# TIXhjq/ML_Function

Hardware: AMD Instinct MI355X
Metric: samples/sec fwd+bwd xDeepFM-CIN B=4096,F=39,K=16 (higher is better)
Workload: dtype f32

## Files before the change

ml_function_amd/csrc/cin.hip:

```cpp
#include "cin_layout.h"

namespace fil {

static const char* kFwdNames[kCinMaxL] = {"cin_fwd_l1", "cin_fwd_l2", "cin_fwd_l3", "cin_fwd_l4", "cin_fwd_l5", "cin_fwd_l6", "cin_fwd_l7", "cin_fwd_l8"};
static const char* kDwNames[kCinMaxL] = {"cin_bwd_dw_l1", "cin_bwd_dw_l2", "cin_bwd_dw_l3", "cin_bwd_dw_l4", "cin_bwd_dw_l5", "cin_bwd_dw_l6", "cin_bwd_dw_l7", "cin_bwd_dw_l8"};
static const char* kDzNames[kCinMaxL] = {"cin_bwd_dz_l1", "cin_bwd_dz_l2", "cin_bwd_dz_l3", "cin_bwd_dz_l4", "cin_bwd_dz_l5", "cin_bwd_dz_l6", "cin_bwd_dz_l7", "cin_bwd_dz_l8"};
static double gemm_flops(long M, int Hp, int F, int H) { return 2.0 * (double)M * Hp * F * H; }

static int launch_dw3(hipStream_t st, const DwPlan& p, const float* gT, int HS, const float* xT, const float* xpT, int xps, float* part,
                      long M, int F, int Hp, int H, int symD = 0, int xtra = 0) {
  const int items = p.blocks_x * p.splits * p.chunks;
  const dim3 grid((items + 7) / 8 * 8);
#define FIL_DW3(MBV, ONES) \
  hipLaunchKernelGGL((cin_dw3_kernel<MBV, ONES>), grid, dim3(kCinThreads), 0, st, gT, HS, xT, xpT, xps, part, (int)M, F, Hp, H, p.rows_per_split, \
                     p.blocks_x, p.chunks, items, symD, xtra)
  if (xT == nullptr) {
    if (p.MB == 2) FIL_DW3(2, true); else FIL_DW3(1, true);
  } else {
    if (p.MB == 2) FIL_DW3(2, false); else FIL_DW3(1, false);
  }
#undef FIL_DW3
  return p.splits;
}

constexpr int kCinRetiredBits = 0;
static bool tail_used(const CinShape& s, int mode) {
  if ((mode & (FIL_CIN_GENERAL | FIL_CIN_NOTAIL)) != 0) return false;
  const TailGeom g = tail_geom(s);
  if (!g.on) return false;
  return (mode & FIL_CIN_TAIL_ALWAYS) != 0 || 4 * g.JP <= 3 * g.Hq;
}
static bool qtail_used(const CinShape& s, int mode, const CinTune& tune) {
  if (s.M() <= 16384 && (mode & FIL_CIN_TAIL_ALWAYS) == 0) return false;
  return tail_used(s, mode) && s.L == 3 && tune.sym && s.F >= 2 && s.F + 2 <= kQtConst && s.H[0] <= 128 && 3 * s.F + 1 <= s.HSmax() && (mode & FIL_CIN_NOQTAIL) == 0 &&
         knobs().qtail != 0;
}
static bool qmerge_used(const CinShape& s, int mode, const CinTune& tune) {
  return qtail_used(s, mode, tune) && 3 * s.F + 3 <= s.HSmax() && (mode & FIL_CIN_NOQMERGE) == 0 && knobs().qmerge != 0;
}
constexpr int kCinPrecBf16 = 1 << 20;
static bool qsplit_fwd_menu(int JT) { return JT >= 2 && JT <= 12 && JT % 2 == 0; }
static bool qsplit_used(const CinShape& s, int mode, const CinTune& tune) {
  return (mode & (FIL_CIN_BF16X3 | kCinPrecBf16)) != 0 && qmerge_used(s, mode, tune) && knobs().fwdq != 0 && knobs().dz2 != 0 && s.HS(0) == 128 &&
         qsplit_fwd_menu(cin_jt_sym(s.F));
}

struct CinPath {
  bool xt_in;
  bool general;
  bool tail;
  bool qtail;
  bool qmerge;
  bool qsplit;
  int qnp;
  CinTune tune;
  TailGeom tg;
  bool fwdq(const CinShape& s) const { return qmerge && knobs().fwdq != 0 && s.HS(0) == 128; }
};
static CinPath cin_path_of(const CinShape& s, int mode) {
  const CinTune tune(mode);
  return CinPath{(mode & FIL_CIN_X_TRANSPOSED) != 0, (mode & FIL_CIN_GENERAL) != 0, tail_used(s, mode), qtail_used(s, mode, tune), qmerge_used(s, mode, tune),
                 qsplit_used(s, mode, tune), (mode & kCinPrecBf16) != 0 ? 1 : 3, tune, tail_geom(s)};
}
static int cin_precision_bits(const char* who, int mode, int precision, int* bits) {
  if (precision != FIL_CIN_PREC_DEFAULT && precision != FIL_CIN_PREC_BF16)
    return fail(FIL_ERR_ARG, "%s: precision %d (0 DEFAULT, 1 BF16)", who, precision);
  if (precision == FIL_CIN_PREC_BF16 && (mode & FIL_CIN_BF16X3) != 0)
    return fail(FIL_ERR_ARG, "%s: precision BF16 with mode bit BF16X3 (mode %d): two operand precisions", who, mode);
  *bits = precision == FIL_CIN_PREC_BF16 ? kCinPrecBf16 : 0;
  return FIL_OK;
}
static int cin_path(const char* who, const CinShape& s, int mode, int precision, CinPath* path) {
  if (mode < 0 || mode > 1023 || (mode & kCinRetiredBits) != 0)
    return fail(FIL_ERR_UNSUPPORTED, "%s: mode %d (bits: 1 general kernels, 2 BF16X3, 4 MB2, 8 NOSYM, 16 X_TRANSPOSED, 32 NOTAIL, 64 TAIL_ALWAYS, 128 NOKSPLIT, 256 NOQTAIL, 512 NOQMERGE)", who, mode);
  int bits = 0;
  if (int rc = cin_precision_bits(who, mode, precision, &bits)) return rc;
  *path = cin_path_of(s, mode | bits);
  return FIL_OK;
}
static int cin_ready_order(int L, const CinPath& p, int* slot, int* point) {
  int n = 0, pt = 0;
  slot[n] = L, point[n++] = pt;
  if (p.qmerge) slot[n] = 0, point[n++] = pt;
  ++pt;
  int l = L - 1;
  if (p.tail) {
    slot[n] = L - 1, point[n++] = pt;
    slot[n] = L - 2, point[n++] = pt++;
    l = L - 3;
  }
  for (; l >= (p.qmerge ? 1 : 0); --l) slot[n] = l, point[n++] = pt++;
  return pt;
}
static SavedForm saved_form(const CinPath& p) { return p.qtail ? SavedForm::qtail : (p.tail ? SavedForm::tail : SavedForm::plain); }

template <typename KernelT>
static void allow_lds(KernelT kernel, size_t sh) {
  if (sh > 48 * 1024) (void)hipFuncSetAttribute(reinterpret_cast<const void*>(kernel), hipFuncAttributeMaxDynamicSharedMemorySize, (int)sh);
}

struct DzsShape {
  int MBs, ks;
  dim3 grid;
};
static DzsShape dzs_launch_shape(const CinTune& tune, long M, int JTs, int NHMAX) {
  const bool two_waves = NHMAX == 64 && cin_dzs_two_waves(JTs) && tune.mb_forced != 2 && knobs().dzs_mb != 2;
  const int MBs = (two_waves || NHMAX == 128) ? 1 : tune.mb_rows(M);
  const int ks = (NHMAX != 64 || MBs != 1) ? 1 : tune.ksplit(M);
  return DzsShape{MBs, ks, dim3(ks == 4 ? cdiv((int)M, 32) : cdiv((int)M, 128 * MBs))};
}

}

using namespace fil;

extern "C" size_t fil_cin_saved_bytes(int B, int F, int K, int L, const int* H) {
  CinShape s;
  if (check_shape("fil_cin_saved_bytes", B, F, K, L, H, s) != FIL_OK || B == 0) return 0;
  return saved_bytes(s);
}

extern "C" size_t fil_cin_fwd_workspace_bytes(int B, int F, int K, int L, const int* H) {
  CinShape s;
  if (check_shape("fil_cin_fwd_workspace_bytes", B, F, K, L, H, s) != FIL_OK || B == 0) return 0;
  return fwd_ws_bytes(s);
}

extern "C" size_t fil_cin_bwd_workspace_bytes(int B, int F, int K, int L, const int* H) {
  CinShape s;
  if (check_shape("fil_cin_bwd_workspace_bytes", B, F, K, L, H, s) != FIL_OK || B == 0) return 0;
  return bwd_ws_bytes(s);
}

extern "C" int fil_cin_grad_ready_points(int B, int F, int K, int L, const int* H, int mode, int* point) {
  CinShape s;
  if (int rc = check_shape("fil_cin_grad_ready_points", B, F, K, L, H, s)) return rc;
  if (point == nullptr || mode < 0 || mode > 1023) return fail(FIL_ERR_ARG, "fil_cin_grad_ready_points: point == NULL or mode %d out of range", mode);
  if ((mode & kCinRetiredBits) != 0) return fail(FIL_ERR_UNSUPPORTED, "fil_cin_grad_ready_points: mode %d holds a retired bit (2: the split-bf16 experiment)", mode);
  if (B == 0) {
    for (int i = 0; i <= L; ++i) point[i] = 0;
    return 1;
  }
  int slot[kCinMaxL + 1], pt[kCinMaxL + 1];
  const int n = cin_ready_order(L, cin_path_of(s, mode), slot, pt);
  for (int i = 0; i <= L; ++i) point[slot[i]] = pt[i];
  return n;
}

extern "C" int fil_cin_precision_used(int B, int F, int K, int L, const int* H, int mode, int precision) {
  CinShape s;
  if (int rc = check_shape("fil_cin_precision_used", B, F, K, L, H, s)) return rc;
  if (mode < 0 || mode > 1023 || (mode & kCinRetiredBits) != 0) return fail(FIL_ERR_UNSUPPORTED, "fil_cin_precision_used: mode %d", mode);
  int bits = 0;
  if (int rc = cin_precision_bits("fil_cin_precision_used", mode, precision, &bits)) return rc;
  if (bits == 0 || B == 0) return FIL_CIN_PREC_DEFAULT;
  return cin_path_of(s, mode | bits).qsplit ? FIL_CIN_PREC_BF16 : FIL_CIN_PREC_DEFAULT;
}

#define FIL_CIN_CHECK_ARG(cond)                                                          \
  do {                                                                                   \
    if (!(cond)) return ::fil::fail(FIL_ERR_ARG, "%s: bad argument: %s", c.who, #cond); \
  } while (0)
#define FIL_CIN_FWD_LAUNCHED() FIL_CHECK_LAUNCH_W("cin_fwd_impl")
#define FIL_CIN_BWD_LAUNCHED() FIL_CHECK_LAUNCH_W("cin_bwd_impl")

struct CinCall {
  const char* who;
  CinShape s;
  CinPath p;
  hipStream_t st;
  const float* x;
  const float* xT;
  const float* const* W;
  const float* const* bias;
  const float* dense_w;
  int output_dim;
  CinSaved sv;
};
struct CinFwd : CinCall {
  const float* dense_b;
  float *out, *pooled;
  CinFwdWs ws;
  PoolArgs pa;
  const float* xpT;
  bool fused_last = false;
  bool head_done = false;
};

static int cin_fwd_prepare(CinFwd& c) {
  const CinShape& s = c.s;
  const TailGeom& tg = c.p.tg;
  const int B = s.B, F = s.F, K = s.K, L = s.L, JT = s.JT(), XL = cin_x2_len(F);
  const long M = s.M();
  const bool xt_in = c.p.xt_in, need_x2 = c.p.tune.sym;
  hipStream_t st = c.st;
  if (c.p.qtail) {
    FIL_CIN_CHECK_ARG(c.W[0] && c.W[L - 1] && c.W[L - 2]);
    ProfScope ps("cin_fwd_prep", st, 2.0 * M * F * sizeof(float));
    const int JTs = cin_jt_sym(F), chunks0 = chunks_of(s.H[0]);
    const long npack = (long)chunks0 * F * 2 * JTs * 128;
    const bool fq = c.p.fwdq(s);
    const int nt = fq ? 0 : B, npk = (int)std::min<long>((npack + 255) / 256, 1024), nwl = cdiv(tg.Hq * F, 8), nwp = cdiv(tg.Hpp * F, 8);
    const size_t sh = (xt_in || fq) ? 0 : (size_t)F * (K + 1) * sizeof(float);
    allow_lds(cin_qtail_prep_kernel, sh);
    hipLaunchKernelGGL(cin_qtail_prep_kernel, dim3(nt + npk + nwl + nwp), dim3(256), sh, st, c.x, c.sv.xT, F, K, nt, c.W[0], c.ws.Wf, s.H[0], 2 * JTs, chunks0, npk,
                       c.W[L - 1], c.sv.wsumL, tg.Hq, tg.HL, nwl, c.W[L - 2], c.sv.wsumP, c.sv.wsnP, tg.Hpp, 2 * JT, chunks_of(tg.Hpp), c.ws.x2T, XL, xt_in ? 1 : 0);
  } else if (c.p.tail && c.p.tune.sym) {
    FIL_CIN_CHECK_ARG(c.W[0] && c.W[L - 1]);
    ProfScope ps("cin_fwd_prep", st, 2.0 * M * F * sizeof(float));
    const int JTs = cin_jt_sym(F), chunks0 = chunks_of(s.H[0]);
    const long npack = (long)chunks0 * F * 2 * JTs * 128;
    const int nt = B, npk = (int)std::min<long>((npack + 255) / 256, 1024), nws = cdiv(tg.Hq * F, 8), nz = 64;
    const size_t sh = xt_in ? 0 : (size_t)F * (K + 1) * sizeof(float);
    allow_lds(cin_fwd_prep_kernel, sh);
    hipLaunchKernelGGL(cin_fwd_prep_kernel, dim3(nt + npk + nws + nz), dim3(256), sh, st, c.x, c.sv.xT, F, K, nt, c.W[0], c.ws.Wf, s.H[0], 2 * JTs, chunks0,
                       npk, c.W[L - 1], c.sv.bmT, tg.Hq, tg.HL, nws, reinterpret_cast<float4*>(c.sv.Uz), (long)((tg.uz_floats + tg.uf_floats) / 4), c.ws.x2T, XL,
                       xt_in ? 1 : 0);
  } else if (!xt_in || need_x2) {
    ProfScope ps("cin_transpose_in", st, 2.0 * M * F * sizeof(float));
    hipLaunchKernelGGL(cin_transpose_in_kernel, dim3(B), dim3(256), xt_in ? 0 : (size_t)F * (K + 1) * sizeof(float), st, c.x, c.sv.xT, F, K,
                       need_x2 ? c.ws.x2T : nullptr, XL, xt_in ? 1 : 0);
  }
  FIL_CIN_FWD_LAUNCHED();
  return FIL_OK;
}

static int cin_fwd_merged_q(CinFwd& c) {
  const CinShape& s = c.s;
  const TailGeom& tg = c.p.tg;
  const CinSaved& sv = c.sv;
  const CinFwdWs& ws = c.ws;
  const int B = s.B, F = s.F, K = s.K, L = s.L, JT = s.JT(), XL = cin_x2_len(F), *H = s.H;
  const long M = s.M();
  const bool xt_in = c.p.xt_in, qsplit = c.p.qsplit;
  const float* x = c.x;
  hipStream_t st = c.st;
  const int p = tg.p, lL = L - 1, Hpp = tg.Hpp, Hq = tg.Hq, HS0 = s.HS(0);
  FIL_CIN_CHECK_ARG(c.W[p] && c.W[lL] && c.bias[p] && c.bias[lL]);
  const int JTs = cin_jt_sym(F), chunks = chunks_of(Hpp);
  float* x1T = sv.maps[0];
  {
    ProfScope ps("cin_tail_prep", st);
    int ks = -1;
    if (!xt_in && K <= 64 && (K & (K - 1)) == 0 && (reinterpret_cast<uintptr_t>(x) & 15) == 0)
      for (ks = 0; (1 << ks) < K;) ++ks;
    const size_t sh_x = ks >= 0 ? (size_t)(64 >> ks) * F * (K + 1) : (xt_in ? (size_t)64 * (F | 1) : (size_t)F * (K + 1));
    const int tiles = cin_slot_tiles(F, JTs);
    const bool fold = !qsplit && knobs().packfold != 0;
    const QtPackFold pf = fold ? QtPackFold{ws.WfT, sv.WzT, JTs, chunks, HS0, tiles} : QtPackFold{nullptr, nullptr, 0, 0, 0, 0};
    const size_t sh = std::max(cin_qtail_t_lds_floats(F, Hq, fold), sh_x) * sizeof(float);
    allow_lds(cin_qtail_t_x_kernel, sh);
    const int nx = (ks >= 0 || xt_in) ? (int)((M + 63) / 64) : B, nT = cin_qtail_t_wgs(Hpp);
    hipLaunchKernelGGL(cin_qtail_t_x_kernel, dim3(nT + nx), dim3(256), sh, st, c.W[p], sv.wsumL, c.bias[p], c.bias[lL], tg.HL, sv.T, sv.cvec, ws.zbias, Hpp, F, Hq,
                       nT, x, sv.xT, K, ws.x2T, XL, xt_in ? 1 : 0, ks, (ks >= 0 || xt_in) ? (long)M : 0L, pf);
    if (!fold) {
      const long npack = (long)chunks * F * 2 * JTs * 128;
      const int nbf = (int)std::min<long>((npack + 255) / 256, 1024), nbz = (int)std::min<long>(((long)tiles * 32 * HS0 + 255) / 256, 1024);
      const int NTq = qsplit ? cin_qs_steps(F, JTs) : 0, nbq = qsplit ? std::min(cdiv(NTq * 512, 256), 512) : 0;
      if (c.p.qnp == 1)
        hipLaunchKernelGGL(cin_qtail_pack_kernel<1>, dim3(nbf + nbz + nbq), dim3(256), 0, st, sv.T, ws.WfT, sv.WzT, F, Hpp, JTs, chunks, nbf, HS0, tiles, nbz,
                           c.W[0], H[0], ws.Wb, NTq);
      else
        hipLaunchKernelGGL(cin_qtail_pack_kernel<3>, dim3(nbf + nbz + nbq), dim3(256), 0, st, sv.T, ws.WfT, sv.WzT, F, Hpp, JTs, chunks, nbf, HS0, tiles, nbz,
                           c.W[0], H[0], ws.Wb, NTq);
    }
  }
  FIL_CIN_FWD_LAUNCHED();
  {
    const double algo = gemm_flops(M, F, F, H[0]) + gemm_flops(M, Hpp, F, Hq) + gemm_flops(M, Hq, F, tg.HL);
    ProfScope ps("cin_fwd_q", st, algo, gemm_flops(M, 1, F * (F / 2 + 1), H[0]) + gemm_flops(M, 1, F * (F / 2 + 1), Hpp));
    CinHeadFold hf{};
    if (K <= 32 && (K & (K - 1)) == 0 && knobs().headfold != 0) {
      int ks = 0;
      while ((1 << ks) < K) ++ks;
      hf = CinHeadFold{c.pooled, c.output_dim == 1 ? c.out : nullptr, c.dense_w, c.dense_b, ks, (int)(L * K), p * K, lL * K};
      c.head_done = true;
    }
    if (qsplit) {
      const int NT = cin_qs_steps(F, JTs);
      if (!cin_launch_fwdq_b(st, c.p.qnp, JTs, ws.x2T, XL, ws.Wb, NT, c.bias[0], sv.wsnP, JT, sv.cvec, x1T, sv.R, HS0, ws.pool[0], ws.pool[p], ws.pool[lL], (int)M, F,
                             H[0], hf))
        return fail(FIL_ERR_UNSUPPORTED, "fil_cin_fwd: no split-bf16 forward kernel for JT=%d (F=%d)", JTs, F);
    } else if (!cin_launch_fwdq(st, JTs, ws.x2T, XL, ws.Wf, ws.WfT, c.bias[0], sv.wsnP, JT, sv.cvec, x1T, sv.R, HS0, ws.pool[0], ws.pool[p], ws.pool[lL], (int)M, F,
                                H[0], hf))
      return fail(FIL_ERR_UNSUPPORTED, "fil_cin_fwd: no merged forward kernel for JT=%d (F=%d)", JTs, F);
    c.pa.chunks[0] = c.pa.chunks[p] = c.pa.chunks[lL] = 1;
  }
  FIL_CIN_FWD_LAUNCHED();
  return FIL_OK;
}

static int cin_fwd_qtail(CinFwd& c, int l) {
  const CinShape& s = c.s;
  const TailGeom& tg = c.p.tg;
  const CinSaved& sv = c.sv;
  const CinFwdWs& ws = c.ws;
  const int F = s.F, L = s.L, JT = s.JT(), XL = cin_x2_len(F), MB = c.p.tune.mb_rows(s.M());
  const long M = s.M();
  const float *xT = c.xT, *xpT = c.xpT;
  hipStream_t st = c.st;
  const int lL = L - 1, Hpp = tg.Hpp, Hq = tg.Hq, HS0 = s.HS(0);
  FIL_CIN_CHECK_ARG(c.W[lL] && c.bias[lL]);
  const int JTs = cin_jt_sym(F), chunks = chunks_of(Hpp);
  {
    ProfScope ps("cin_tail_prep", st);
    const size_t sh = cin_qtail_t_lds_floats(F, Hq, false) * sizeof(float);
    allow_lds(cin_qtail_t_kernel, sh);
    hipLaunchKernelGGL(cin_qtail_t_kernel, dim3(cin_qtail_t_wgs(Hpp)), dim3(256), sh, st, c.W[l], sv.wsumL, c.bias[l], c.bias[lL], tg.HL, sv.T, sv.cvec, ws.zbias, Hpp, F, Hq);
    const long npack = (long)chunks * F * 2 * JTs * 128;
    const int tiles = cin_slot_tiles(F, JTs);
    const int nbf = (int)std::min<long>((npack + 255) / 256, 1024), nbz = (int)std::min<long>(((long)tiles * 32 * HS0 + 255) / 256, 1024);
    hipLaunchKernelGGL(cin_qtail_pack_kernel<3>, dim3(nbf + nbz), dim3(256), 0, st, sv.T, ws.Wf, sv.WzT, F, Hpp, JTs, chunks, nbf, HS0, tiles);
  }
  FIL_CIN_FWD_LAUNCHED();
  {
    const double algo = gemm_flops(M, Hpp, F, Hq) + gemm_flops(M, Hq, F, tg.HL);
    ProfScope ps("cin_fwd_tail", st, algo, gemm_flops(M, 1, F * (F / 2 + 1), Hpp));
    const int ks = c.p.tune.ksplit(M);
    cin_launch_fwd3_sym(st, MB, JTs, dim3(ks == 4 ? cdiv((int)M, 32) : cdiv((int)M, 128 * MB), chunks), xT, ws.x2T, XL, ws.Wf, ws.zbias, sv.R, HS0, ws.pool[lL],
                        (int)M, F, Hpp, ks);
  }
  FIL_CIN_FWD_LAUNCHED();
  {
    ProfScope ps("cin_tail_pool", st);
    const float* wsn = sv.wsnP;
    float *pp = ws.pool[l], *pL = ws.pool[lL];
    const dim3 grid((int)((M + 127) / 128));
#define FIL_QP(JTV) \
  case JTV: hipLaunchKernelGGL((cin_qtail_pool2_kernel<JTV>), grid, dim3(256), 0, st, xT, xpT, s.xps(l), wsn, sv.R, HS0, sv.cvec, pp, pL, (int)M, F, Hpp); break;
    switch (JT) { FIL_QP(4) FIL_QP(8) FIL_QP(12) FIL_QP(16) FIL_QP(20) FIL_QP(24) FIL_QP(28) FIL_QP(32) }
#undef FIL_QP
    c.pa.chunks[l] = c.pa.chunks[lL] = 1;
  }
  FIL_CIN_FWD_LAUNCHED();
  return FIL_OK;
}

static int cin_fwd_fused_tail(CinFwd& c, int l) {
  const CinShape& s = c.s;
  const TailGeom& tg = c.p.tg;
  const CinSaved& sv = c.sv;
  const int F = s.F, lL = s.L - 1, JT = s.JT();
  const long M = s.M();
  hipStream_t st = c.st;
  FIL_CIN_CHECK_ARG(c.W[lL] && c.bias[lL]);
  {
    ProfScope ps("cin_tail_prep", st);
    if (!c.p.tune.sym) {
      hipLaunchKernelGGL(cin_tail_wsum_kernel, dim3(cdiv(tg.Hq * F, 8)), dim3(256), 0, st, c.W[lL], sv.bmT, tg.Hq, F, tg.HL);
      (void)hipMemsetAsync(sv.Uz, 0, (tg.uz_floats + tg.uf_floats) * sizeof(float), st);
    }
    const size_t sh = (size_t)(F + 1) * (((tg.Hq + 3) & ~3) + 4) * sizeof(float);
    allow_lds(cin_tail_ueff_kernel, sh);
    hipLaunchKernelGGL(cin_tail_ueff_kernel, dim3(cdiv(tg.C1, kTailUc)), dim3(256), sh, st, c.W[l], c.bias[l], sv.bmT, c.bias[lL], tg.HL, sv.Uf, sv.Uz, sv.consts,
                       tg.Hpp, F, tg.Hq, tg.JT4, tg.JP, JT, tg.JHp);
  }
  FIL_CIN_FWD_LAUNCHED();
  {
    const double algo = gemm_flops(M, tg.Hpp, F, tg.Hq) + gemm_flops(M, tg.Hq, F, tg.HL);
    ProfScope ps("cin_fwd_tail", st, algo, 2.0 * (double)M * tg.Cp * (F + 1));
    const int RB = c.p.tune.mb_rows(M) == 2 ? 4 : 2;
    TailFwdArgs a{c.xT, c.xpT, s.xps(l), sv.Uf, sv.consts, sv.Y, tg.JP, c.ws.pool[l], c.ws.pool[lL], (int)M, F, tg.Hpp, c.p.tune.ksplit(M)};
    cin_launch_tail_fwd(st, RB, tg.JT4, tg.NCB, a);
    c.pa.chunks[l] = c.pa.chunks[lL] = 1;
  }
  FIL_CIN_FWD_LAUNCHED();
  return FIL_OK;
}

static int cin_fwd_general_layer(CinFwd& c, int l) {
  const CinShape& s = c.s;
  const CinTune& tune = c.p.tune;
  const CinFwdWs& ws = c.ws;
  const int F = s.F, L = s.L, JT = s.JT(), XL = cin_x2_len(F), MB = tune.mb_rows(s.M()), *H = s.H;
  const long M = s.M();
  const float *xT = c.xT, *xpT = c.xpT;
  hipStream_t st = c.st;
  const int Hp = s.Hp(l), Hl = H[l], xps = s.xps(l);
  float* xoutT = l + 1 < L ? c.sv.maps[l] : nullptr;
  float* part = ws.pool[l];
  const bool fuse_next = !c.p.general && l == L - 2 && !(l == 0 && tune.sym);
  if (l == L - 1 && !c.p.general) {
    if (!c.fused_last) {
      const size_t sh = (size_t)Hp * ((F + 3) & ~3) * sizeof(float);
      ProfScope ps("cin_last_fwd", st, 2.0 * (double)M * Hp * F);
      hipLaunchKernelGGL(cin_wsum_kernel, dim3(cdiv(Hp * F, 8)), dim3(256), 0, st, c.W[l], ws.wsum, Hp * F, Hl);
      allow_lds(cin_last_fwd_kernel, sh);
      hipLaunchKernelGGL(cin_last_fwd_kernel, dim3(cdiv((int)M, kLastRows)), dim3(256), sh, st, xT, xpT, xps, ws.wsum, c.bias[l], part, (int)M, F, Hp, Hl);
      c.pa.chunks[l] = 1;
    }
  } else {
    const int chunks = chunks_of(Hl);
    if (l == 0 && tune.sym) {
      const int JTs = cin_jt_sym(F);
      const long npack = (long)chunks * F * 2 * JTs * 128;
      if (!c.p.tail)
        hipLaunchKernelGGL(cin_pack_wf_sym_kernel, dim3((int)std::min<long>((npack + 255) / 256, 2048)), dim3(256), 0, st, c.W[l], ws.Wf, F, Hl, 2 * JTs, chunks);
      ProfScope ps(kFwdNames[l], st, gemm_flops(M, Hp, F, Hl), gemm_flops(M, 1, F * (F / 2 + 1), Hl));
      const int ks = tune.ksplit(M);
      cin_launch_fwd3_sym(st, MB, JTs, dim3(ks == 4 ? cdiv((int)M, 32) : cdiv((int)M, 128 * MB), chunks), xT, ws.x2T, XL, ws.Wf, c.bias[l], xoutT, s.HS(l), part,
                          (int)M, F, Hl, ks);
    } else {
      const long npack = (long)chunks * Hp * 2 * JT * 128;
      hipLaunchKernelGGL(cin_pack_wf_kernel, dim3((int)std::min<long>((npack + 255) / 256, 2048)), dim3(256), 0, st, c.W[l], ws.Wf, Hp, F, Hl, 2 * JT, chunks);
      const float* wsn = nullptr;
      if (fuse_next) {
        FIL_CIN_CHECK_ARG(c.W[l + 1] && c.bias[l + 1]);
        float* wsn_buf = ws.Wf + (size_t)npack;
        hipLaunchKernelGGL(cin_wsum_wsn_kernel, dim3(cdiv(Hl * F, 8)), dim3(256), 0, st, c.W[l + 1], ws.wsum, Hl * F, H[l + 1], wsn_buf, Hl, F, 2 * JT,
                           chunks);
        wsn = wsn_buf;
        c.pa.chunks[l + 1] = chunks;
        c.fused_last = true;
      }
      ProfScope ps(kFwdNames[l], st, gemm_flops(M, Hp, F, Hl) + (fuse_next ? 2.0 * (double)M * Hl * F : 0.0));
      cin_launch_fwd3(st, MB, JT, dim3(cdiv((int)M, 128 * MB), chunks), xT, xpT, xps, ws.Wf, c.bias[l], xoutT, s.HS(l), part, (int)M, F, Hp, Hl,
                      wsn, fuse_next ? c.bias[l + 1] : nullptr, fuse_next ? H[l + 1] : 0, fuse_next ? ws.pool[l + 1] : nullptr);
    }
  }
  FIL_CIN_FWD_LAUNCHED();
  c.xpT = xoutT;
  return FIL_OK;
}

static int cin_fwd_head(CinFwd& c) {
  const int B = c.s.B, K = c.s.K, L = c.s.L;
  if (!c.head_done) {
    ProfScope ps("cin_head_fwd", c.st);
    hipLaunchKernelGGL(cin_head_fwd_kernel, dim3(cdiv(B, kHeadSamples)), dim3(256), (size_t)kHeadSamples * L * K * sizeof(float), c.st, c.pa, c.dense_w, c.dense_b,
                       c.pooled, c.output_dim == 1 ? c.out : nullptr, B, K, L);
  }
  FIL_CIN_FWD_LAUNCHED();
  return FIL_OK;
}

static int cin_fwd_impl(const char* who, const float* x, const float* const* W, const float* const* bias, const float* dense_w,
                        const float* dense_b, float* out, float* pooled, float* saved, int B, int F, int K, int L,
                        const int* H, int output_dim, int mode, int precision, void* workspace, size_t workspace_bytes, void* stream) {
  CinFwd c{};
  c.who = who;
  int rc = check_shape(who, B, F, K, L, H, c.s);
  if (rc != FIL_OK) return rc;
  if ((rc = cin_path(who, c.s, mode, precision, &c.p)) != FIL_OK) return rc;
  if (B == 0) return FIL_OK;
  FIL_CIN_CHECK_ARG(x && W && bias && pooled && saved);
  FIL_CIN_CHECK_ARG(output_dim != 1 || (dense_w && dense_b && out));
  const size_t need = fwd_ws_bytes(c.s);
  if (workspace == nullptr || workspace_bytes < need) return fail(FIL_ERR_WORKSPACE, "fil_cin_fwd: workspace %zu < %zu bytes", workspace_bytes, need);
  c.st = (hipStream_t)stream;
  c.x = x, c.W = W, c.bias = bias, c.dense_w = dense_w, c.dense_b = dense_b, c.out = out, c.pooled = pooled, c.output_dim = output_dim;
  LayoutCarver wsc(workspace), svc(saved);
  c.ws.lay_out(wsc, c.s);
  c.sv.lay_out(svc, c.s, c.p.tg, saved_form(c.p));
  for (int l = 0; l < L; ++l) c.pa.part[l] = c.ws.pool[l], c.pa.chunks[l] = chunks_of(H[l]);
  c.xT = c.xpT = c.p.xt_in ? x : c.sv.xT;
  if ((rc = cin_fwd_prepare(c)) != FIL_OK) return rc;
  const int ltail = !c.p.tail ? L : (c.p.fwdq(c.s) ? 0 : c.p.tg.p);
  for (int l = 0; l < L && rc == FIL_OK; ++l) {
    FIL_CIN_CHECK_ARG(W[l] && bias[l]);
    if (l < ltail) rc = cin_fwd_general_layer(c, l);
    else rc = c.p.fwdq(c.s) ? cin_fwd_merged_q(c) : (c.p.qtail ? cin_fwd_qtail(c, l) : cin_fwd_fused_tail(c, l));
    if (l == ltail) break;
  }
  return rc != FIL_OK ? rc : cin_fwd_head(c);
}

extern "C" int fil_cin_fwd(const float* x, const float* const* W, const float* const* bias, const float* dense_w,
                           const float* dense_b, float* out, float* pooled, float* saved, int B, int F, int K, int L,
                           const int* H, int output_dim, int mode, void* workspace, size_t workspace_bytes, void* stream) {
  return cin_fwd_impl("fil_cin_fwd", x, W, bias, dense_w, dense_b, out, pooled, saved, B, F, K, L, H, output_dim, mode, FIL_CIN_PREC_DEFAULT, workspace,
                      workspace_bytes, stream);
}

extern "C" int fil_cin_fwd_p(const float* x, const float* const* W, const float* const* bias, const float* dense_w,
                             const float* dense_b, float* out, float* pooled, float* saved, int B, int F, int K, int L,
                             const int* H, int output_dim, int mode, int precision, void* workspace, size_t workspace_bytes, void* stream) {
  return cin_fwd_impl("fil_cin_fwd_p", x, W, bias, dense_w, dense_b, out, pooled, saved, B, F, K, L, H, output_dim, mode, precision, workspace,
                      workspace_bytes, stream);
}

struct CinBwd : CinCall {
  const float *pooled, *g;
  float* dx;
  float* const* dW;
  float* const* dbias;
  float *ddense_w, *ddense_b;
  void* const* events;
  CinBwdWs ws;
  const float* dPsrc;
  int nblk, ncol, ndc;
  int ready_slot[kCinMaxL + 1];
  int nready = 0;
  int cur = 0;
  int ltop;
  bool dx_started = false;
  bool have_gx0 = false;
  bool wz_prepacked = false;
  bool qm_joined = false;
};

static void cin_record_ready(const CinBwd& c, int slot) {
  if (c.events != nullptr && c.events[slot] != nullptr) (void)hipEventRecord((hipEvent_t)c.events[slot], c.st);
}
static void ready_next(CinBwd& c) { cin_record_ready(c, c.ready_slot[c.nready++]); }

static int cin_bwd_head(CinBwd& c) {
  const int B = c.s.B, LK = c.s.L * c.s.K;
  hipStream_t st = c.st;
  c.dPsrc = c.g;
  if (c.output_dim == 1 && c.p.qmerge) {
    c.dPsrc = c.ws.dP;
  } else if (c.output_dim == 1) {
    ProfScope ps("cin_head_bwd", st);
    hipLaunchKernelGGL(cin_head_bwd_kernel, dim3(c.nblk), dim3(256), 0, st, c.g, c.dense_w, c.pooled, c.ws.dP, c.ws.small, B, LK, kHeadChunk);
    if (!c.p.tail)
      hipLaunchKernelGGL(cin_reduce_kernel, dim3(cdiv(LK + 1, 64)), dim3(256), 0, st, c.ws.small, c.ddense_w, (long)(LK + 1), c.nblk, c.ddense_b, (long)LK);
    FIL_CIN_BWD_LAUNCHED();
    c.dPsrc = c.ws.dP;
  }
  if (!c.p.tail) ready_next(c);
  return FIL_OK;
}

static void cin_qtail_params_fill(const CinBwd& c) {
  const TailGeom& tg = c.p.tg;
  const CinBwdWs& ws = c.ws;
  const int F = c.s.F, p = tg.p, lL = c.s.L - 1, Hpp = tg.Hpp, Hq = tg.Hq;
  ProfScope ps("cin_tail_params", c.st);
  const size_t sh = cin_qtail_params_lds(F, Hq);
  allow_lds(cin_qtail_params_kernel, sh);
  float* dcfin = ws.dcpart + (size_t)c.ndc * kQtConst;
  hipLaunchKernelGGL(cin_qtail_params_kernel, dim3(2 * Hpp + 1), dim3(256), sh, c.st, c.W[p], c.sv.wsumL, ws.dT, ws.vlast, c.dW[p], ws.part, Hpp, F, Hq, ws.dcpart, c.ndc,
                     dcfin);
  hipLaunchKernelGGL(cin_qtail_fill_kernel, dim3(cdiv(Hq * F, kQtFillCols)), dim3(kQtFillThreads), 0, c.st, ws.part, Hpp, dcfin, c.bias[p], c.sv.wsumL, c.dW[lL], c.dbias[p],
                     c.dbias[lL], F, Hq, tg.HL);
}

static int cin_bwd_top_merged_q(CinBwd& c) {
  const CinShape& s = c.s;
  const TailGeom& tg = c.p.tg;
  const CinSaved& sv = c.sv;
  const CinBwdWs& ws = c.ws;
  const int F = s.F, K = s.K, L = s.L, JT = s.JT(), LK = s.L * s.K, *H = s.H;
  const long M = s.M();
  const bool qsplit = c.p.qsplit;
  const float* xT = c.xT;
  hipStream_t st = c.st;
  const int p = tg.p, lL = L - 1, Hpp = tg.Hpp, Hq = tg.Hq, HS0 = s.HS(0);
  FIL_CIN_CHECK_ARG(c.bias && c.W[0] && c.W[p] && c.W[lL] && c.bias[p] && c.dW[0] && c.dW[p] && c.dW[lL] && c.dbias[0] && c.dbias[p] && c.dbias[lL]);
  const float* xpT = sv.maps[p - 1];
  const int xps = s.xps(p);
  const float* dPp = c.dPsrc + (size_t)p * K;
  const float* dPL = c.dPsrc + (size_t)lL * K;
  const float* dPprev = c.dPsrc + (size_t)(p - 1) * K;
  const double algo_tail = gemm_flops(M, Hpp, F, Hq) + gemm_flops(M, Hq, F, tg.HL);
  const double algo1 = gemm_flops(M, F, F, H[0]);
  const int symD = F / 2 + 1, Cl = F * symD;
  const int JTs = cin_jt_sym(F);
  const int periods = cin_dz_periods(F, JTs), tiles0 = cin_slot_tiles(F, JTs);
  const CinBwdWs::Scratch v = ws.scratch(s, true);
  float* G = ws.G[c.cur];
  {
    ProfScope ps("cin_tail_a", st, (double)M * (2 * F + 3) * sizeof(float));
    const size_t sh = (size_t)256 * (F + 3 + (c.output_dim == 1 ? L : 0)) * sizeof(float);
    allow_lds(cin_qtail_xe_kernel<3>, sh);
    allow_lds(cin_qtail_xe_kernel<1>, sh);
    const int np = (int)std::min<long>(((long)tiles0 * 32 * HS0 + 255) / 256, 1024);
    const int nq2 = qsplit ? 2 * std::min(cdiv(tiles0 * 512, 256), 256) : 0;
    if (c.p.qnp == 1)
      hipLaunchKernelGGL(cin_qtail_xe_kernel<1>, dim3(c.ndc + np + nq2), dim3(kXeThreads), sh, st, xT, dPL, dPp, LK, K, v.xr, ws.dcpart, (int)M, F,
                         c.ndc, c.output_dim == 1 ? c.g : nullptr, c.dense_w, c.pooled, ws.dP, ws.hpart, LK, lL, p, c.W[0], ws.Wz, H[0], JTs, HS0, tiles0, np, sv.T,
                         Hpp, ws.Wzb1, ws.Wzb2);
    else
      hipLaunchKernelGGL(cin_qtail_xe_kernel<3>, dim3(c.ndc + np + nq2), dim3(kXeThreads), sh, st, xT, dPL, dPp, LK, K, v.xr, ws.dcpart, (int)M, F,
                         c.ndc, c.output_dim == 1 ? c.g : nullptr, c.dense_w, c.pooled, ws.dP, ws.hpart, LK, lL, p, c.W[0], ws.Wz, H[0], JTs, HS0, tiles0, np, sv.T,
                         Hpp, ws.Wzb1, ws.Wzb2);
  }
  FIL_CIN_BWD_LAUNCHED();
  {
    ProfScope ps("cin_last_bwd", st, 6.0 * (double)M * Hpp * F);
    cin_launch_last_bwd2(st, JT, xT, xpT, xps, sv.wsumP, sv.wsnP, dPp, LK, dPprev, G, HS0, ws.dxT, (int)M, F, K, Hpp, sv.R, HS0, dPL, ws.small);
  }
  FIL_CIN_BWD_LAUNCHED();
  int dw_parts = 0;
  {
    ProfScope ps("cin_bwd_dw_q", st, algo1 + algo_tail, gemm_flops(M, 1, Cl, H[0]) + gemm_flops(M, 1, Cl, Hpp));
    if (qsplit) {
      const DwqbPlan bp = cin_dwqb_plan(M, Cl + F, cu_count());
      cin_launch_dwq_b(st, c.p.qnp, bp, G, xpT, HS0, v.xr, v.XS, ws.part, (int)M, F, symD);
      dw_parts = bp.splits;
    } else {
      const bool f4 = knobs().dwfold4 != 0;
      const DwqPlan dp = f4 ? cin_dwq_plan4(M, Cl + F, cu_count()) : cin_dwq_plan(M, Cl + F, cu_count());
      if (f4)
        hipLaunchKernelGGL((cin_dwq_kernel<kDwqDepth, 4>), dim3((dp.wgs + 7) / 8 * 8), dim3(kDwqThreads), 0, st, G, xpT, HS0, v.xr, v.XS, ws.part, (int)M, F,
                           symD, dp.rows_per_split, dp.splits, dp.ncol_full, dp.rem, dp.wgs_full, dp.wgs);
      else
        hipLaunchKernelGGL((cin_dwq_kernel<kDwqDepth, 2>), dim3((dp.wgs + 7) / 8 * 8), dim3(kDwqThreads), 0, st, G, xpT, HS0, v.xr, v.XS, ws.part, (int)M, F,
                           symD, dp.rows_per_split, dp.splits, dp.ncol_full, dp.rem, dp.wgs_full, dp.wgs);
      dw_parts = dp.pairs;
    }
  }
  FIL_CIN_BWD_LAUNCHED();
  {
    ProfScope ps("cin_reduce_dw", st);
    const int nb1 = cdiv(H[0], 64);
    const int nh = c.output_dim == 1 ? cdiv(LK + 1, 64) : 0;
    hipLaunchKernelGGL(cin_reduce_expand_q_kernel, dim3((Cl + F + 3) / 4 + nb1 + nh), dim3(256), 0, st, ws.part, dw_parts, F, symD, H[0], Hpp, c.dW[0], ws.dT,
                       ws.vlast, ws.small, c.ncol, c.dbias[0], nb1, ws.hpart, c.ndc, LK, c.ddense_w, c.ddense_b);
  }
  FIL_CIN_BWD_LAUNCHED();
  ready_next(c);
  ready_next(c);
  cin_qtail_params_fill(c);
  FIL_CIN_BWD_LAUNCHED();
  ready_next(c);
  ready_next(c);
  const int NHMAX = HS0 / 2;
  if (NHMAX == 64 && knobs().dz2 != 0) {
    ProfScope ps("cin_bwd_dz_q", st, algo1 + algo_tail, gemm_flops(M, 1, Cl, H[0]) + gemm_flops(M, 1, Cl, Hpp));
    bool split_done = false;
    if (qsplit) {
      split_done = cin_launch_dz2_b(st, c.p.qnp, JTs, G, xpT, HS0, dPL, LK, K, ws.Wzb1, ws.Wzb2, xT, ws.dxT, 1, (int)M, F, H[0], Hpp, periods, c.dx, sv.cvec);
    }
    if (!split_done &&
        !cin_launch_dz2(st, JTs, G, xpT, HS0, dPL, LK, K, ws.Wz, sv.WzT, xT, ws.dxT, 1, (int)M, F, H[0], Hpp, periods, c.dx, sv.cvec))
      return fail(FIL_ERR_UNSUPPORTED, "fil_cin_bwd: no two-pass data-gradient kernel for JT=%d (F=%d)", JTs, F);
    c.qm_joined = true;
  } else {
    const DzsShape z = dzs_launch_shape(c.p.tune, M, JTs, NHMAX);
    {
      ProfScope ps("cin_bwd_dz_tail", st, algo_tail, gemm_flops(M, 1, Cl, Hpp));
      cin_launch_dz3_sym(st, z.MBs, JTs, NHMAX, z.grid, xpT, HS0, sv.WzT, xT, v.gxR, v.dxR, 0, (int)M, F, Hpp, periods, z.ks);
    }
    FIL_CIN_BWD_LAUNCHED();
    {
      ProfScope ps("cin_bwd_dz_l1", st, algo1, gemm_flops(M, 1, Cl, H[0]));
      cin_launch_dz3_sym(st, z.MBs, JTs, NHMAX, z.grid, G, HS0, ws.Wz, xT, ws.gx0T, ws.dxT, 1, (int)M, F, H[0], periods, z.ks);
    }
    c.have_gx0 = true;
  }
  FIL_CIN_BWD_LAUNCHED();
  c.dx_started = true;
  c.ltop = -1;
  return FIL_OK;
}

static int cin_bwd_top_qtail(CinBwd& c) {
  const CinShape& s = c.s;
  const TailGeom& tg = c.p.tg;
  const CinSaved& sv = c.sv;
  const CinBwdWs& ws = c.ws;
  const int F = s.F, K = s.K, L = s.L, JT = s.JT(), LK = s.L * s.K, *H = s.H;
  const long M = s.M();
  const float* xT = c.xT;
  hipStream_t st = c.st;
  const int p = tg.p, lL = L - 1, Hpp = tg.Hpp, Hq = tg.Hq, HS0 = s.HS(0);
  FIL_CIN_CHECK_ARG(c.bias && c.W[p] && c.W[lL] && c.bias[p] && c.dW[p] && c.dW[lL] && c.dbias[p] && c.dbias[lL]);
  const float* xpT = sv.maps[p - 1];
  const int xps = s.xps(p);
  const float* dPp = c.dPsrc + (size_t)p * K;
  const float* dPL = c.dPsrc + (size_t)lL * K;
  const float* dPprev = c.dPsrc + (size_t)(p - 1) * K;
  const double algo = gemm_flops(M, Hpp, F, Hq) + gemm_flops(M, Hq, F, tg.HL);
  const int symD = F / 2 + 1, Cl = F * symD;
  const int JTs = cin_jt_sym(F);
  const CinBwdWs::Scratch v = ws.scratch(s, false);
  {
    ProfScope ps("cin_tail_a", st, (double)M * (F + 64) * sizeof(float));
    const size_t sh = (size_t)256 * (F + 3) * sizeof(float);
    allow_lds(cin_qtail_scale_kernel, sh);
    const int nh = c.output_dim == 1 ? cdiv(LK + 1, 64) : 0;
    FIL_CIN_CHECK_ARG(c.W[0]);
    const int tiles0 = cin_slot_tiles(F, JTs);
    const int np = (int)std::min<long>(((long)tiles0 * 32 * HS0 + 255) / 256, 1024);
    hipLaunchKernelGGL(cin_qtail_scale_kernel, dim3(c.ndc + nh + np), dim3(256), sh, st, xT, dPL, dPp, LK, K, v.xr, ws.dcpart, (int)M, F, c.ndc, ws.small,
                       c.ddense_w, c.ddense_b, LK, c.nblk, nh, c.W[0], ws.Wz, H[0], JTs, HS0, tiles0);
    c.wz_prepacked = true;
  }
  FIL_CIN_BWD_LAUNCHED();
  ready_next(c);
  {
    ProfScope ps("cin_last_bwd", st, 6.0 * (double)M * Hpp * F);
    cin_launch_last_bwd2(st, JT, xT, xpT, xps, sv.wsumP, sv.wsnP, dPp, LK, dPprev, ws.G[c.cur], HS0, ws.dxT, (int)M, F, K, Hpp, sv.R, HS0, dPL, ws.small);
  }
  FIL_CIN_BWD_LAUNCHED();
  {
    ProfScope ps("cin_bwd_dw_tail", st, algo, gemm_flops(M, 1, Cl, Hpp));
    const int parts = launch_dw3(st, dw_plan(M, Cl + F, Hpp), xpT, HS0, xT, v.xr, v.XS, ws.part, M, F, F, Hpp, symD, F);
    const long nW = (long)Cl * Hpp, pstride = (long)(Cl + F) * Hpp;
    hipLaunchKernelGGL(cin_reduce_expand_sym_kernel, dim3((int)((nW + 63) / 64) + cdiv(F * Hpp, 64)), dim3(256), 0, st, ws.part, ws.dT, F, symD, Hpp, parts,
                       pstride, ws.vlast, (long)F * Hpp);
  }
  FIL_CIN_BWD_LAUNCHED();
  cin_qtail_params_fill(c);
  FIL_CIN_BWD_LAUNCHED();
  ready_next(c);
  ready_next(c);
  {
    ProfScope ps("cin_bwd_dz_tail", st, algo, gemm_flops(M, 1, Cl, Hpp));
    const int NHMAX = HS0 / 2;
    const DzsShape z = dzs_launch_shape(c.p.tune, M, JTs, NHMAX);
    cin_launch_dz3_sym(st, z.MBs, JTs, NHMAX, z.grid, xpT, HS0, sv.WzT, xT, v.gxR, v.dxR, 0, (int)M, F, Hpp, cin_dz_periods(F, JTs), z.ks);
  }
  FIL_CIN_BWD_LAUNCHED();
  c.dx_started = true;
  c.ltop = p - 1;
  return FIL_OK;
}

static int cin_bwd_top_fused_tail(CinBwd& c) {
  const CinShape& s = c.s;
  const TailGeom& tg = c.p.tg;
  const CinSaved& sv = c.sv;
  const CinBwdWs& ws = c.ws;
  const int F = s.F, K = s.K, L = s.L, JT = s.JT(), LK = s.L * s.K, *H = s.H;
  const long M = s.M();
  const float* xT = c.xT;
  hipStream_t st = c.st;
  const int p = tg.p, lL = L - 1;
  FIL_CIN_CHECK_ARG(c.bias && c.W[p] && c.W[lL] && c.bias[p] && c.dW[p] && c.dW[lL] && c.dbias[p] && c.dbias[lL]);
  const float* xpT = sv.maps[p - 1];
  const int xps = s.xps(p);
  const double algo = gemm_flops(M, tg.Hpp, F, tg.Hq) + gemm_flops(M, tg.Hq, F, tg.HL);
  float* Apk = ws.G[1];
  c.wz_prepacked = p == 1 && c.p.tune.sym && F >= 2;
  {
    ProfScope ps("cin_tail_a", st, (double)M * (F + 64) * sizeof(float));
    const int na = (int)std::min<long>((M * 16 * tg.NCB + 255) / 256, 4096);
    const int nh = c.output_dim == 1 ? cdiv(LK + 1, 64) : 0;
    int np = 0, JTs = 0, tiles0 = 0;
    if (c.wz_prepacked) {
      FIL_CIN_CHECK_ARG(c.W[0]);
      JTs = cin_jt_sym(F);
      tiles0 = cin_slot_tiles(F, JTs);
      np = (int)std::min<long>(((long)tiles0 * 32 * s.HS(0) + 255) / 256, 1024);
    }
    hipLaunchKernelGGL(cin_tail_pre_kernel, dim3(na + nh + np), dim3(256), 0, st, xT, c.dPsrc, LK, K, p, lL, Apk, (int)M, F, tg.NCB, na, ws.small,
                       c.ddense_w, c.ddense_b, LK, c.nblk, nh, c.W[0], ws.Wz, H[0], JTs, s.HS(0), tiles0);
  }
  FIL_CIN_BWD_LAUNCHED();
  ready_next(c);
  const TailDwPlan tp = tail_dw_plan(M, tg.C1);
  {
    ProfScope ps("cin_bwd_dw_tail", st, algo, 2.0 * (double)M * tg.C1 * (F + 2));
    TailDwArgs a{Apk, xT, xpT, xps, ws.part, (int)M, F, tg.Hpp, tg.JP, tp.rows_per_split, tp.blocks_x, tp.blocks_x * tp.splits, knobs().tail_settle != 0};
    cin_launch_tail_dw(st, tg.NCB, a);
  }
  FIL_CIN_BWD_LAUNCHED();
  {
    ProfScope ps("cin_tail_params", st);
    const int nblk_p = cdiv(tg.Cp, kTailPc);
    const int ldb = (tg.Hq + 3) & ~3;
    const size_t sh = ((size_t)(F + 1) * ldb + (size_t)tg.JP * (kTailPc + 4) + (size_t)kTailPc * ldb) * sizeof(float);
    allow_lds(cin_tail_params_kernel, sh);
    float* partB = ws.part + (size_t)tp.splits * tg.C1 * tg.JP;
    float* qones = ws.vlast;
    hipLaunchKernelGGL(cin_tail_params_kernel, dim3(2 * nblk_p), dim3(256), sh, st, ws.part, tp.splits, c.W[p], sv.bmT, c.dW[p], c.dbias[p], partB, qones,
                       tg.Cp, F, tg.Hq, tg.JP);
    hipLaunchKernelGGL(cin_tail_fill_kernel, dim3(cdiv(tg.Hq * F, 64)), dim3(256), 0, st, partB, nblk_p, qones, c.bias[p], c.dW[lL], c.dbias[lL], F,
                       tg.Hq, tg.HL);
  }
  FIL_CIN_BWD_LAUNCHED();
  ready_next(c);
  ready_next(c);
  {
    ProfScope ps("cin_bwd_dz_tail", st, algo, 2.0 * (double)M * tg.Cp * (F + 1));
    TailDzArgs a{sv.Uz, xT, xpT, xps, sv.Y, tg.JP, c.dPsrc, LK, K, p, lL, ws.G[c.cur], s.HS(p - 1), ws.dxT, (int)M, F, tg.Hpp, tg.periods, knobs().tail_dz_mode,
                 c.p.tune.ksplit(M)};
    cin_launch_tail_dz(st, JT, tg.NQ, a);
  }
  FIL_CIN_BWD_LAUNCHED();
  c.dx_started = true;
  c.ltop = p - 1;
  return FIL_OK;
}

static int cin_bwd_top_shortcut(CinBwd& c) {
  const CinShape& s = c.s;
  const CinBwdWs& ws = c.ws;
  const int B = s.B, F = s.F, K = s.K, L = s.L, JT = s.JT(), LK = s.L * s.K, nblk = c.nblk;
  const long M = s.M();
  const float* xT = c.xT;
  hipStream_t st = c.st;
  const int l = L - 1;
  FIL_CIN_CHECK_ARG(c.W[l] && c.dW[l] && c.dbias[l]);
  const int Hp = s.Hp(l), Hl = s.H[l], xps = s.xps(l);
  const size_t cl = (size_t)Hp * F;
  const float* xpT = l == 0 ? xT : c.sv.maps[l - 1];
  const float* dPl = c.dPsrc + (size_t)l * K;
  const float* dPprev = l > 0 ? c.dPsrc + (size_t)(l - 1) * K : nullptr;
  const size_t shw = (size_t)Hp * ((F + 3) & ~3) * sizeof(float);
  ProfScope ps("cin_last_bwd", st, 6.0 * (double)M * Hp * F);
  hipLaunchKernelGGL(cin_wsum_wsn_kernel, dim3(cdiv(Hp * F, 8)), dim3(256), 0, st, c.W[l], ws.wsum, Hp * F, Hl, l > 0 ? ws.Wz : nullptr, Hp, F, 2 * JT,
                     chunks_of(Hp));
  hipLaunchKernelGGL(cin_slice_sum_kernel, dim3(nblk), dim3(256), 0, st, dPl, LK, ws.small, B, K, kHeadChunk);
  {
    float* yT = ws.G[1];
    const int YS = (F + 3) & ~3;
    const long tot = M * YS;
    hipLaunchKernelGGL(cin_scale_rows3_kernel, dim3((int)std::min<long>((tot + 255) / 256, 4096)), dim3(256), 0, st, xT, dPl, LK, K, yT, (int)M, F, YS);
    const bool swap = l > 0;
    int nb;
    if (swap) nb = launch_dw3(st, dw_plan(M, F, Hp), xpT, xps, nullptr, yT, YS, ws.part, M, 1, F, Hp);
    else nb = launch_dw3(st, dw_plan(M, Hp, F), yT, YS, nullptr, xpT, xps, ws.part, M, 1, Hp, F);
    hipLaunchKernelGGL(cin_reduce_kernel, dim3(cdiv((int)cl, 64)), dim3(256), 0, st, ws.part, ws.vlast, (long)cl, nb);
    hipLaunchKernelGGL(cin_fill_rows_kernel, dim3((int)std::min<long>(((long)cl * Hl + 255) / 256, 2048)), dim3(256), 0, st, ws.vlast, c.dW[l], (long)cl, Hl,
                       swap ? F : 0, Hp, ws.small, nblk, c.dbias[l]);
  }
  ready_next(c);
  if (l > 0) {
    cin_launch_last_bwd2(st, JT, xT, xpT, xps, ws.wsum, ws.Wz, dPl, LK, dPprev, ws.G[c.cur], s.HS(l - 1), ws.dxT, (int)M, F, K, Hp);
  } else {
    const size_t shb = shw + (size_t)kLastRows * (kLastFMax + 1) * sizeof(float);
    allow_lds(cin_last_bwd_kernel, shb);
    hipLaunchKernelGGL(cin_last_bwd_kernel, dim3(cdiv((int)M, kLastRows)), dim3(256), shb, st, xT, xpT, xps, ws.wsum, dPl, LK, dPprev,
                       nullptr, 0, ws.dxT, 1, (int)M, F, K, Hp);
  }
  FIL_CIN_BWD_LAUNCHED();
  c.dx_started = true;
  c.ltop = L - 2;
  return FIL_OK;
}

static int cin_bwd_top_bcast(CinBwd& c) {
  const CinShape& s = c.s;
  const int L = s.L, LK = s.L * s.K;
  const long total = s.M() * s.HS(L - 1);
  ProfScope ps("cin_bcast_g", c.st, (double)total * sizeof(float));
  hipLaunchKernelGGL(cin_bcast3_kernel, dim3((int)std::min<long>((total + 255) / 256, 4096)), dim3(256), 0, c.st, c.dPsrc + (size_t)(L - 1) * s.K, LK,
                     s.K, c.ws.G[c.cur], s.HS(L - 1), (int)s.M(), s.H[L - 1]);
  FIL_CIN_BWD_LAUNCHED();
  c.ltop = L - 1;
  return FIL_OK;
}

static int cin_bwd_general_layer(CinBwd& c, int l) {
  const CinShape& s = c.s;
  const CinTune& tune = c.p.tune;
  const CinBwdWs& ws = c.ws;
  const int F = s.F, K = s.K, JT = s.JT(), LK = s.L * s.K, ncol = c.ncol;
  const long M = s.M();
  const float* xT = c.xT;
  hipStream_t st = c.st;
  FIL_CIN_CHECK_ARG(c.W[l] && c.dW[l] && c.dbias[l]);
  const int Hp = s.Hp(l), Hl = s.H[l], HSl = s.HS(l), xps = s.xps(l);
  const float* xpT = l == 0 ? xT : c.sv.maps[l - 1];
  const float* G = ws.G[c.cur];
  {
    ProfScope ps("cin_dbias", st, (double)M * Hl * sizeof(float));
    if (!(c.p.qtail && l == c.ltop)) hipLaunchKernelGGL(cin_colsum3_kernel, dim3(ncol), dim3(256), 0, st, G, HSl, ws.small, (int)M, Hl, kColRows);
    hipLaunchKernelGGL(cin_reduce_kernel, dim3(cdiv(Hl, 64)), dim3(256), 0, st, ws.small, c.dbias[l], (long)Hl, ncol);
  }
  FIL_CIN_BWD_LAUNCHED();
  int parts;
  const int symD = (l == 0 && tune.sym) ? F / 2 + 1 : 0;
  const int Cl = symD > 0 ? F * symD : Hp * F;
  {
    ProfScope ps(kDwNames[l], st, gemm_flops(M, Hp, F, Hl), gemm_flops(M, 1, Cl, Hl));
    parts = launch_dw3(st, dw_plan(M, Cl, Hl), G, HSl, xT, xpT, xps, ws.part, M, F, Hp, Hl, symD);
  }
  FIL_CIN_BWD_LAUNCHED();
  const long nW = (long)Cl * Hl;
  {
    ProfScope ps("cin_reduce_dw", st, (double)(parts + 1) * nW * sizeof(float));
    if (symD > 0) hipLaunchKernelGGL(cin_reduce_expand_sym_kernel, dim3((int)((nW + 63) / 64)), dim3(256), 0, st, ws.part, c.dW[l], F, symD, Hl, parts);
    else hipLaunchKernelGGL(cin_reduce_kernel, dim3((int)((nW + 63) / 64)), dim3(256), 0, st, ws.part, c.dW[l], nW, parts);
  }
  FIL_CIN_BWD_LAUNCHED();
  ready_next(c);
  {
    const int NHMAX = HSl / 2;
    const int MBg = NHMAX == 128 ? 1 : ((knobs().dz_mb == 2 && JT <= 28) ? 2 : 1);
    const float* dPprev = l > 0 ? c.dPsrc + (size_t)(l - 1) * K : nullptr;
    if (l == 0 && tune.sym && F >= 2) {
      const int JTs = cin_jt_sym(F);
      const int tiles = cin_slot_tiles(F, JTs);
      const long npack = (long)tiles * 32 * HSl;
      if (!c.wz_prepacked) {
        hipLaunchKernelGGL(cin_pack_wz_sym_kernel, dim3((int)std::min<long>((npack + 255) / 256, 2048)), dim3(256), 0, st, c.W[l], ws.Wz, F, Hl, JTs, HSl, tiles);
      }
      ProfScope ps(kDzNames[l], st, gemm_flops(M, Hp, F, Hl), gemm_flops(M, 1, F * (F / 2 + 1), Hl));
      const DzsShape z = dzs_launch_shape(tune, M, JTs, NHMAX);
      cin_launch_dz3_sym(st, z.MBs, JTs, NHMAX, z.grid, G, HSl, ws.Wz, xT, ws.gx0T, ws.dxT, c.dx_started ? 1 : 0, (int)M, F, Hl, cin_dz_periods(F, JTs), z.ks);
    } else {
      const int periods = cin_dz_periods(Hp, JT), tiles = cin_slot_tiles(Hp, JT);
      const long npack = (long)tiles * 32 * HSl;
      hipLaunchKernelGGL(cin_pack_wz_kernel, dim3((int)std::min<long>((npack + 255) / 256, 2048)), dim3(256), 0, st, c.W[l], ws.Wz, Hp, F, Hl, JT, HSl, tiles);
      ProfScope ps(kDzNames[l], st, gemm_flops(M, Hp, F, Hl));
      cin_launch_dz3(st, MBg, JT, NHMAX, dim3(cdiv((int)M, 128 * MBg)), G, HSl, ws.Wz, xT, xpT, xps, dPprev, LK, K,
                     l > 0 ? ws.G[c.cur ^ 1] : nullptr, l > 0 ? s.HS(l - 1) : 0, l == 0 ? ws.gx0T : nullptr, ws.dxT, c.dx_started ? 1 : 0,
                     (int)M, F, Hp, Hl, periods);
    }
    c.dx_started = true;
    if (l == 0) c.have_gx0 = true;
  }
  FIL_CIN_BWD_LAUNCHED();
  c.cur ^= 1;
  return FIL_OK;
}

static int cin_bwd_finish_dx(CinBwd& c) {
  const CinShape& s = c.s;
  const int F = s.F, K = s.K, LK = s.L * s.K;
  if (!c.qm_joined) {
    ProfScope ps("cin_transpose_out", c.st, 2.0 * s.M() * F * sizeof(float));
    const float* gx0T = c.have_gx0 ? c.ws.gx0T : nullptr;
    if (c.p.qtail) {
      const CinBwdWs::Scratch v = c.ws.scratch(s, c.p.qmerge);
      hipLaunchKernelGGL(cin_transpose_out_kernel, dim3(s.B), dim3(256), (size_t)K * (F + 1) * sizeof(float), c.st, c.ws.dxT, gx0T, c.dx, F, K, v.gxR, v.dxR,
                         c.sv.cvec, c.dPsrc + (size_t)(s.L - 1) * K, LK);
    } else {
      hipLaunchKernelGGL(cin_transpose_out_kernel, dim3(s.B), dim3(256), (size_t)K * (F + 1) * sizeof(float), c.st, c.ws.dxT, gx0T, c.dx, F, K);
    }
  }
  FIL_CIN_BWD_LAUNCHED();
  return FIL_OK;
}

static int cin_bwd_impl(const char* who, const float* x, const float* const* W, const float* const* bias, const float* dense_w,
                        const float* pooled, const float* saved, const float* g, float* dx, float* const* dW,
                        float* const* dbias, float* ddense_w, float* ddense_b, int B, int F, int K, int L, const int* H,
                        int output_dim, int mode, int precision, void* const* grad_ready_events, void* workspace, size_t workspace_bytes,
                        void* stream) {
  CinBwd c{};
  c.who = who;
  int rc = check_shape(who, B, F, K, L, H, c.s);
  if (rc != FIL_OK) return rc;
  if ((rc = cin_path(who, c.s, mode, precision, &c.p)) != FIL_OK) return rc;
// ... 56 lines not shown
```

ml_function_amd/csrc/cin_kernels.h:

```cpp
#pragma once
#include "common.h"

namespace fil {

constexpr int kCinThreads = 256;
constexpr int kCinMaxL = 8;
constexpr int kCinMaxH = 256;

__device__ __forceinline__ f32x16 mfma32(float a, float b, f32x16 c) {
  return __builtin_amdgcn_mfma_f32_32x32x2f32(a, b, c, 0, 0, 0);
}

__device__ __forceinline__ void settle(float& v) { asm volatile("" : "+v"(v)); }
typedef float f32x4s __attribute__((ext_vector_type(4)));
__device__ __forceinline__ void settle(f32x4s& v) { asm volatile("" : "+v"(v)); }

__device__ __forceinline__ __amdgpu_buffer_rsrc_t make_rsrc(const float* p, long bytes) {
  return __builtin_amdgcn_make_buffer_rsrc(const_cast<float*>(p), 0, (int)std::min<long>(bytes, 0x7fffffffL), 0x00020000);
}
__device__ __forceinline__ __amdgpu_buffer_rsrc_t make_rsrc_uniform(const float* p, long bytes) {
  const unsigned long a = reinterpret_cast<unsigned long>(p);
  const unsigned lo = __builtin_amdgcn_readfirstlane((unsigned)a), hi = __builtin_amdgcn_readfirstlane((unsigned)(a >> 32));
  const int n = __builtin_amdgcn_readfirstlane((int)std::min<long>(bytes, 0x7fffffffL));
  return __builtin_amdgcn_make_buffer_rsrc(reinterpret_cast<float*>(((unsigned long)hi << 32) | lo), 0, n, 0x00020000);
// ... 945 lines not shown
  const long total = (long)M * HS;
  for (long i = (long)blockIdx.x * blockDim.x + threadIdx.x; i < total; i += (long)gridDim.x * blockDim.x) {
    const long m = i / HS;
    const int n = (int)(i - m * HS);
    const long b = m / K;
    gT[i] = n < H ? dP[b * ldp + (m - b * K)] : 0.f;
  }
}

static __global__ __launch_bounds__(256) void cin_scale_rows3_kernel(const float* __restrict__ xT, const float* __restrict__ dP, int ldp, int K,
                                                              float* __restrict__ yT, int M, int F, int YS) {
  const long total = (long)M * YS;
  for (long i = (long)blockIdx.x * blockDim.x + threadIdx.x; i < total; i += (long)gridDim.x * blockDim.x) {
    const long m = i / YS;
    const int f = (int)(i - m * YS);
    const long b = m / K;
    yT[i] = f < F ? xT[m * F + f] * dP[b * ldp + (m - b * K)] : 0.f;
  }
}

__device__ __forceinline__ void cin_reduce_body(const float* __restrict__ part, float* __restrict__ out, long n, int parts,
                                                float* __restrict__ out2, long n1, int bid, long pstride = 0) {
  __shared__ float red[4][64];
  const int lane = threadIdx.x & 63, wave = threadIdx.x >> 6;
  const long i = (long)bid * 64 + lane;
  const long ps = pstride > 0 ? pstride : n;
  float t0 = 0.f, t1 = 0.f, t2 = 0.f, t3 = 0.f;
  if (i < n) {
    int p = wave;
    for (; p + 60 < parts; p += 64) {
      float u[16];
#pragma unroll
      for (int e = 0; e < 16; ++e) u[e] = part[(long)(p + 4 * e) * ps + i];
#pragma unroll
      for (int e = 0; e < 16; e += 4) {
        t0 += u[e];
        t1 += u[e + 1];
        t2 += u[e + 2];
        t3 += u[e + 3];
      }
    }
    for (; p + 12 < parts; p += 16) {
      t0 += part[(long)p * ps + i];
      t1 += part[(long)(p + 4) * ps + i];
      t2 += part[(long)(p + 8) * ps + i];
      t3 += part[(long)(p + 12) * ps + i];
    }
    for (; p < parts; p += 4) t0 += part[(long)p * ps + i];
  }
  red[wave][lane] = (t0 + t1) + (t2 + t3);
  __syncthreads();
  if (wave == 0 && i < n) {
    const float v = (red[0][lane] + red[1][lane]) + (red[2][lane] + red[3][lane]);
    if (out2 != nullptr && i >= n1) out2[i - n1] = v;
    else out[i] = v;
  }
}
static __global__ __launch_bounds__(256) void cin_reduce_kernel(const float* __restrict__ part, float* __restrict__ out, long n,
                                                         int parts, float* __restrict__ out2 = nullptr, long n1 = 0, long pstride = 0) {
  cin_reduce_body(part, out, n, parts, out2, n1, blockIdx.x, pstride);
}

static __global__ __launch_bounds__(256) void cin_reduce_expand_sym_kernel(const float* __restrict__ part, float* __restrict__ dW, int F, int D,
                                                                    int H, int parts, long pstride = 0, float* __restrict__ vout = nullptr,
                                                                    long nv = 0) {
  if (vout != nullptr) {
    const long nbw = ((long)F * D * H + 63) / 64;
    if ((long)blockIdx.x >= nbw) {
      cin_reduce_body(part + (long)F * D * H, vout, nv, parts, nullptr, 0, (int)(blockIdx.x - nbw), pstride);
      return;
    }
  }
  __shared__ float red[4][64];
  const int lane = threadIdx.x & 63, wave = threadIdx.x >> 6;
  const long n = (long)F * D * H;
  const long ps = pstride > 0 ? pstride : n;
  const long i = (long)blockIdx.x * 64 + lane;
  float t0 = 0.f, t1 = 0.f, t2 = 0.f, t3 = 0.f;
  if (i < n) {
    int p = wave;
    for (; p + 60 < parts; p += 64) {
      float u[16];
#pragma unroll
      for (int e = 0; e < 16; ++e) u[e] = part[(long)(p + 4 * e) * ps + i];
#pragma unroll
      for (int e = 0; e < 16; e += 4) {
        t0 += u[e];
        t1 += u[e + 1];
        t2 += u[e + 2];
        t3 += u[e + 3];
      }
    }
    for (; p + 12 < parts; p += 16) {
      t0 += part[(long)p * ps + i];
      t1 += part[(long)(p + 4) * ps + i];
      t2 += part[(long)(p + 8) * ps + i];
      t3 += part[(long)(p + 12) * ps + i];
    }
    for (; p < parts; p += 4) t0 += part[(long)p * ps + i];
  }
  red[wave][lane] = (t0 + t1) + (t2 + t3);
  __syncthreads();
  if (wave == 0 && i < n) {
    const float v = (red[0][lane] + red[1][lane]) + (red[2][lane] + red[3][lane]);
    const int col = (int)(i % H);
    const int pair = (int)(i / H);
    const int h = pair / D, d = pair - h * D;
    const int f = (h + d) % F;
    dW[((long)h * F + f) * H + col] = v;
    if (d != 0 && 2 * d != F) dW[((long)f * F + h) * H + col] = v;
  }
}

static __global__ __launch_bounds__(256) void cin_slice_sum_kernel(const float* __restrict__ dP, int ldp, float* __restrict__ part, int B,
                                                            int K, int bchunk) {
  __shared__ float red[256];
  const int b_lo = blockIdx.x * bchunk, b_hi = min(B, b_lo + bchunk);
  float t = 0.f;
  const int total = (b_hi - b_lo) * K;
  for (int i = threadIdx.x; i < total; i += 256) {
    const int b = b_lo + i / K, k = i % K;
    t += dP[(long)b * ldp + k];
  }
  red[threadIdx.x] = t;
  __syncthreads();
  for (int s = 128; s > 0; s >>= 1) {
    if (threadIdx.x < s) red[threadIdx.x] += red[threadIdx.x + s];
    __syncthreads();
  }
  if (threadIdx.x == 0) part[blockIdx.x] = red[0];
}

constexpr int kLastFMax = 64;

static __global__ __launch_bounds__(256) void cin_wsum_kernel(const float* __restrict__ W, float* __restrict__ wsum, int C, int H) {
  const int row = blockIdx.x * 8 + (threadIdx.x >> 5), l = threadIdx.x & 31;
  float t = 0.f;
  if (row < C)
    for (int n = l; n < H; n += 32) t += W[(long)row * H + n];
  t = half_wave_sum(t);
  if (row < C && l == 0) wsum[row] = t;
}

static __global__ __launch_bounds__(256) void cin_wsum_wsn_kernel(const float* __restrict__ W, float* __restrict__ wsum, int C, int H,
                                                           float* __restrict__ wsn, int Hp, int F, int JT2, int chunks) {
  const int row = blockIdx.x * 8 + (threadIdx.x >> 5), l = threadIdx.x & 31;
  float t = 0.f;
  if (row < C)
    for (int n = l; n < H; n += 32) t += W[(long)row * H + n];
  t = half_wave_sum(t);
  if (row < C && l == 0) {
    wsum[row] = t;
    if (wsn != nullptr) {
      const int n = row / F, fp = row - n * F;
      wsn[(((n >> 7) * JT2) + fp) * 128 + (n & 127)] = t;
    }
  }
  if (wsn != nullptr) {
    const int total = chunks * JT2 * 128;
    for (int i = blockIdx.x * blockDim.x + threadIdx.x; i < total; i += gridDim.x * blockDim.x) {
      const int col = i & 127, fp = (i >> 7) % JT2, chunk = (i >> 7) / JT2;
      if (fp >= F || chunk * 128 + col >= Hp) wsn[i] = 0.f;
    }
  }
}

__device__ __forceinline__ void stage_wsum(const float* __restrict__ wsum, float* ws, int Hp, int F, int FP4) {
  for (int idx = threadIdx.x; idx < Hp * FP4; idx += blockDim.x) {
    const int h = idx / FP4, f = idx - h * FP4;
    ws[idx] = f < F ? wsum[h * F + f] : 0.f;
  }
}

constexpr int kLastRows = 64;

static __global__ __launch_bounds__(256) void cin_last_fwd_kernel(const float* __restrict__ xT, const float* __restrict__ xpT, int xps,
                                                           const float* __restrict__ wsum, const float* __restrict__ bias,
                                                           float* __restrict__ pool, int M, int F, int Hp, int H) {
  extern __shared__ __attribute__((aligned(16))) float smem[];
  const int FP4 = (F + 3) & ~3;
  stage_wsum(wsum, smem, Hp, F, FP4);
  float bsum = 0.f;
  for (int n = 0; n < H; ++n) bsum += bias[n];
  __syncthreads();
  const int lane = threadIdx.x & 63, wave = threadIdx.x >> 6;
  const int m = blockIdx.x * kLastRows + wave * 16 + (lane & 15), hq = lane >> 4;
  const bool valid = m < M;
  const long mm = valid ? m : 0;
  float xr[kLastFMax];
#pragma unroll
  for (int f = 0; f < kLastFMax; ++f) xr[f] = (valid && f < F) ? xT[mm * F + f] : 0.f;
  const float* xprow = xpT + mm * xps;
  float p = 0.f;
  for (int h = hq; h < Hp; h += 4) {
    const float4* wrow = reinterpret_cast<const float4*>(smem + h * FP4);
    float t = 0.f;
#pragma unroll
    for (int f4 = 0; f4 < kLastFMax / 4; ++f4) {
      if (4 * f4 < F) {
        const float4 w = wrow[f4];
        t = fmaf(xr[4 * f4], w.x, t);
        t = fmaf(xr[4 * f4 + 1], w.y, t);
        t = fmaf(xr[4 * f4 + 2], w.z, t);
        t = fmaf(xr[4 * f4 + 3], w.w, t);
      }
    }
    p = fmaf(valid ? xprow[h] : 0.f, t, p);
  }
  p += __shfl_xor(p, 16);
  p += __shfl_xor(p, 32);
  if (valid && hq == 0) pool[m] = p + bsum;
}

static __global__ __launch_bounds__(256) void cin_last_bwd_kernel(const float* __restrict__ xT, const float* __restrict__ xpT, int xps,
                                                           const float* __restrict__ wsum, const float* __restrict__ dP, int ldp,
                                                           const float* __restrict__ dPprev, float* __restrict__ GprevT, int HSp,
                                                           float* __restrict__ dxT, int layer1, int M, int F, int K, int Hp) {
  extern __shared__ __attribute__((aligned(16))) float smem[];
  const int FP4 = (F + 3) & ~3;
  float* ts = smem + Hp * FP4;
  stage_wsum(wsum, smem, Hp, F, FP4);
  __syncthreads();
  const int lane = threadIdx.x & 63, wave = threadIdx.x >> 6;
  const int rowl = wave * 16 + (lane & 15), hq = lane >> 4;
  const int m = blockIdx.x * kLastRows + rowl;
  const bool valid = m < M;
  const long mm = valid ? m : 0;
  const int b = (int)(mm / K), k = (int)(mm - (long)b * K);
  float xr[kLastFMax], u[kLastFMax];
#pragma unroll
  for (int f = 0; f < kLastFMax; ++f) {
    xr[f] = (valid && f < F) ? xT[mm * F + f] : 0.f;
    u[f] = 0.f;
  }
  const float dp = valid ? dP[(long)b * ldp + k] : 0.f;
  const float dpp = (valid && dPprev != nullptr) ? dPprev[(long)b * ldp + k] : 0.f;
  const float* xprow = xpT + mm * xps;
  for (int h = hq; h < Hp; h += 4) {
    const float4* wrow = reinterpret_cast<const float4*>(smem + h * FP4);
    const float xph = valid ? xprow[h] : 0.f;
    float t = 0.f;
#pragma unroll
    for (int f4 = 0; f4 < kLastFMax / 4; ++f4) {
      if (4 * f4 < F) {
        const float4 w = wrow[f4];
        t = fmaf(xr[4 * f4], w.x, t);
        t = fmaf(xr[4 * f4 + 1], w.y, t);
        t = fmaf(xr[4 * f4 + 2], w.z, t);
        t = fmaf(xr[4 * f4 + 3], w.w, t);
        u[4 * f4] = fmaf(xph, w.x, u[4 * f4]);
        u[4 * f4 + 1] = fmaf(xph, w.y, u[4 * f4 + 1]);
        u[4 * f4 + 2] = fmaf(xph, w.z, u[4 * f4 + 2]);
        u[4 * f4 + 3] = fmaf(xph, w.w, u[4 * f4 + 3]);
      }
    }
    if (layer1) ts[rowl * (kLastFMax + 1) + h] = t;
    else if (valid) GprevT[mm * HSp + h] = fmaf(dp, t, dpp);
  }
  if (layer1) __syncthreads();
#pragma unroll
  for (int f = 0; f < kLastFMax; ++f) {
    if (f < F) {
      float v = u[f];
      v += __shfl_xor(v, 16);
      v += __shfl_xor(v, 32);
      if (layer1) v += ts[rowl * (kLastFMax + 1) + f];
      if (valid && hq == 0) dxT[mm * F + f] = dp * v;
    }
  }
}

static __global__ __launch_bounds__(256) void cin_fill_rows_kernel(const float* __restrict__ v, float* __restrict__ dW, long C, int H, int Ft,
                                                            int Hp, const float* __restrict__ bpart = nullptr, int bparts = 0,
                                                            float* __restrict__ dbias = nullptr) {
  if (bpart != nullptr && blockIdx.x == 0) {
    __shared__ float red[256];
    float t = 0.f;
    for (int p = threadIdx.x; p < bparts; p += 256) t += bpart[p];
    red[threadIdx.x] = t;
    __syncthreads();
    for (int s = 128; s > 0; s >>= 1) {
      if (threadIdx.x < s) red[threadIdx.x] += red[threadIdx.x + s];
      __syncthreads();
    }
    const float tot = red[0];
    for (int n = threadIdx.x; n < H; n += 256) dbias[n] = tot;
  }
  const long total = C * H;
  for (long i = (long)blockIdx.x * blockDim.x + threadIdx.x; i < total; i += (long)gridDim.x * blockDim.x) {
    const long c = i / H;
    dW[i] = Ft > 0 ? v[(c % Ft) * Hp + c / Ft] : v[c];
  }
}

constexpr int kLast2Ld = 66;
constexpr int kLast2Stage = 32 * kLast2Ld;
template <int JT>
__global__ __launch_bounds__(256, 2) void cin_last_bwd2_kernel(const float* __restrict__ xT, const float* __restrict__ xpT, int xps,
                                                            const float* __restrict__ wsum, const float* __restrict__ wsn,
                                                            const float* __restrict__ dP, int ldp, const float* __restrict__ dPprev,
                                                            float* __restrict__ GprevT, int HSp, float* __restrict__ dxT, int M, int F,
                                                            int K, int Hp, const float* __restrict__ Radd = nullptr, int HSr = 0,
                                                            const float* __restrict__ dPadd = nullptr, float* __restrict__ colpart = nullptr) {
  __shared__ float colred[4][128];
  extern __shared__ __attribute__((aligned(16))) float smem[];
  for (int i = threadIdx.x; i < Hp * F; i += 256) smem[i] = wsum[i];
  __syncthreads();
  const int tid = threadIdx.x, lane = tid & 63, wave = tid >> 6;
  const int r = lane & 31, half = lane >> 5;
  const int wrow0 = (blockIdx.x * 4 + wave) * 32;
  if (wrow0 >= M && colpart == nullptr) return;
  const long mq = min(wrow0 + r, M - 1);
  float* stg = smem + ((Hp * F + 3) & ~3) + wave * kLast2Stage;
  const int nrow = min(32, M - wrow0);
  if (nrow > 0) {
    const float4* src = reinterpret_cast<const float4*>(xT + (long)wrow0 * F);
    const int n4 = nrow * F / 4, tail = nrow * F - 4 * n4;
    for (int i = lane; i < n4; i += 64) *reinterpret_cast<float4*>(stg + 4 * i) = src[i];
    if (lane < tail) stg[4 * n4 + lane] = xT[(long)wrow0 * F + 4 * n4 + lane];
  }
  __builtin_amdgcn_wave_barrier();
  float xr[JT];
  {
    const float* xrow = stg + min(r, max(nrow, 1) - 1) * F;
#pragma unroll
    for (int j = 0; j < JT; ++j) {
      const int f = 2 * j + half;
      xr[j] = (f < F && nrow > 0) ? xrow[min(f, F - 1)] : 0.f;
    }
  }
  __shared__ float dps[4][3][32];
  if (half == 0) {
    const int b = (int)(mq / K), k = (int)(mq - (long)b * K);
    dps[wave][0][r] = dP[(long)b * ldp + k];
    dps[wave][1][r] = dPprev != nullptr ? dPprev[(long)b * ldp + k] : 0.f;
    dps[wave][2][r] = Radd != nullptr ? dPadd[(long)b * ldp + k] : 0.f;
  }
  __builtin_amdgcn_wave_barrier();
  auto phase_t = [&]() {
  const int chunks = (Hp + 127) >> 7;
  for (int chunk = 0; chunk < chunks; ++chunk) {
    f32x16 t[4];
#pragma unroll
    for (int nb = 0; nb < 4; ++nb)
#pragma unroll
      for (int i = 0; i < 16; ++i) t[nb][i] = 0.f;
    const float4* wsb = reinterpret_cast<const float4*>(wsn + (long)chunk * (2 * JT) * 128) + (half * 32 + r);
    constexpr int QB = JT % 5 == 0 ? 5 : 4;
#pragma unroll
    for (int j0 = 0; j0 < JT; j0 += QB) {
      float4 wq[QB];
#pragma unroll
      for (int j = 0; j < QB; ++j) wq[j] = wsb[(long)(2 * (j0 + j)) * 32];
      __builtin_amdgcn_sched_barrier(0);
#pragma unroll
      for (int j = 0; j < QB; ++j) {
        const float4 w = wq[j];
        t[0] = mfma32(xr[j0 + j], w.x, t[0]);
        t[1] = mfma32(xr[j0 + j], w.y, t[1]);
        t[2] = mfma32(xr[j0 + j], w.z, t[2]);
        t[3] = mfma32(xr[j0 + j], w.w, t[3]);
      }
    }
    const int n0 = chunk * 128 + 4 * r;
    float c0 = 0.f, c1 = 0.f, c2 = 0.f, c3 = 0.f;
    float4 rq[8];
#pragma unroll
    for (int reg = 0; reg < 16; ++reg) {
      if (Radd != nullptr && (reg & 7) == 0) {
#pragma unroll
        for (int u = 0; u < 8; ++u) {
          const long mm = min(wrow0 + mfma32_row(reg + u, half), M - 1);
          rq[u] = *reinterpret_cast<const float4*>(Radd + mm * HSr + n0);
        }
      }
      const int row = mfma32_row(reg, half);
      const int m = wrow0 + row;
      const float dpr = dps[wave][0][row], dppr = dps[wave][1][row], dpa = dps[wave][2][row];
      if (m < M) {
        float* dst = GprevT + (long)m * HSp + n0;
        float v0 = fmaf(dpr, t[0][reg], dppr), v1 = fmaf(dpr, t[1][reg], dppr);
        float v2 = fmaf(dpr, t[2][reg], dppr), v3 = fmaf(dpr, t[3][reg], dppr);
        if (Radd != nullptr) {
          const float4 ra = rq[reg & 7];
          v0 = fmaf(dpa, ra.x, v0);
          v1 = fmaf(dpa, ra.y, v1);
          v2 = fmaf(dpa, ra.z, v2);
          v3 = fmaf(dpa, ra.w, v3);
        }
        c0 += v0;
        c1 += v1;
        c2 += v2;
        c3 += v3;
        if (n0 + 3 < Hp) {
          *reinterpret_cast<float4*>(dst) = make_float4(v0, v1, v2, v3);
        } else {
          if (n0 < Hp) dst[0] = v0;
          if (n0 + 1 < Hp) dst[1] = v1;
          if (n0 + 2 < Hp) dst[2] = v2;
        }
      }
    }
    if (colpart != nullptr) {
      c0 = lane_halves_sum(c0);
      c1 = lane_halves_sum(c1);
      c2 = lane_halves_sum(c2);
      c3 = lane_halves_sum(c3);
      if (half == 0) *reinterpret_cast<float4*>(&colred[wave][4 * r]) = make_float4(c0, c1, c2, c3);
      __syncthreads();
      for (int n = tid; n < 128; n += 256)
        if (chunk * 128 + n < Hp) colpart[(long)blockIdx.x * Hp + chunk * 128 + n] = (colred[0][n] + colred[1][n]) + (colred[2][n] + colred[3][n]);
      __syncthreads();
    }
  }
  };
  auto phase_u = [&]() {
  if (wrow0 >= M) return;
  f32x16 u0, u1;
#pragma unroll
  for (int i = 0; i < 16; ++i) u0[i] = u1[i] = 0.f;
  const bool two = F > 32;
  const int quads = (Hp + 3) >> 2;
#pragma unroll 1
  for (int q0 = 0; q0 < quads; q0 += 16) {
    __builtin_amdgcn_wave_barrier();
    {
      float4 v[8];
#pragma unroll
      for (int i = 0; i < 8; ++i) {
        const int row = (lane >> 4) + 4 * i, c4 = lane & 15;
        const long mm = min(wrow0 + row, M - 1);
        v[i] = 4 * q0 + 4 * c4 < xps ? *reinterpret_cast<const float4*>(xpT + mm * xps + 4 * q0 + 4 * c4) : make_float4(0.f, 0.f, 0.f, 0.f);
      }
#pragma unroll
      for (int i = 0; i < 8; ++i) {
        const int row = (lane >> 4) + 4 * i, c4 = lane & 15;
        float* d = stg + row * kLast2Ld + 4 * c4;
        *reinterpret_cast<float2*>(d) = make_float2(v[i].x, v[i].y);
        *reinterpret_cast<float2*>(d + 2) = make_float2(v[i].z, v[i].w);
      }
    }
    __builtin_amdgcn_wave_barrier();
    float2 av[16];
    const float* xprow = stg + r * kLast2Ld + 2 * half;
#pragma unroll
    for (int i = 0; i < 16; ++i) av[i] = q0 + i < quads ? *reinterpret_cast<const float2*>(xprow + 4 * i) : make_float2(0.f, 0.f);
#pragma unroll
    for (int i0 = 0; i0 < 16; i0 += 4) {
      float b0[4][2], b1[4][2];
#pragma unroll
      for (int ii = 0; ii < 4; ++ii) {
        const int h = 4 * (q0 + i0 + ii) + 2 * half;
        const float* w0 = smem + min(h, Hp - 1) * F;
        const float* w1 = smem + min(h + 1, Hp - 1) * F;
        const int k0 = (h < Hp && r < F) ? -1 : 0, k1 = (h + 1 < Hp && r < F) ? -1 : 0;
        b0[ii][0] = __builtin_bit_cast(float, __builtin_bit_cast(int, w0[min(r, F - 1)]) & k0);
        b0[ii][1] = __builtin_bit_cast(float, __builtin_bit_cast(int, w1[min(r, F - 1)]) & k1);
        b1[ii][0] = b1[ii][1] = 0.f;
        if (two) {
          const int k2 = (h < Hp && r + 32 < F) ? -1 : 0, k3 = (h + 1 < Hp && r + 32 < F) ? -1 : 0;
          b1[ii][0] = __builtin_bit_cast(float, __builtin_bit_cast(int, w0[min(r + 32, F - 1)]) & k2);
          b1[ii][1] = __builtin_bit_cast(float, __builtin_bit_cast(int, w1[min(r + 32, F - 1)]) & k3);
        }
      }
      __builtin_amdgcn_sched_barrier(0);
#pragma unroll
      for (int ii = 0; ii < 4; ++ii) {
        u0 = mfma32(av[i0 + ii].x, b0[ii][0], u0);
        u0 = mfma32(av[i0 + ii].y, b0[ii][1], u0);
        if (two) {
          u1 = mfma32(av[i0 + ii].x, b1[ii][0], u1);
          u1 = mfma32(av[i0 + ii].y, b1[ii][1], u1);
        }
      }
    }
  }
#pragma unroll
  for (int reg = 0; reg < 16; ++reg) {
    const int m = wrow0 + mfma32_row(reg, half);
    if (m < M) {
      const float dpr = dps[wave][0][mfma32_row(reg, half)];
      if (r < F) dxT[(long)m * F + r] = dpr * u0[reg];
      if (two && r + 32 < F) dxT[(long)m * F + 32 + r] = dpr * u1[reg];
    }
  }
  };
  if ((blockIdx.x >> 3) & 1) {
    phase_u();
    phase_t();
  } else {
    phase_t();
    phase_u();
  }
}

struct PoolArgs {
  const float* part[kCinMaxL];
  int chunks[kCinMaxL];
};

constexpr int kHeadSamples = 8;
static __global__ __launch_bounds__(256) void cin_head_fwd_kernel(PoolArgs pa, const float* __restrict__ dense_w,
                                                           const float* __restrict__ dense_b, float* __restrict__ pooled,
                                                           float* __restrict__ out, int B, int K, int L) {
  extern __shared__ float sh[];
  const int LK = L * K;
  const long M = (long)B * K;
  const int b0 = blockIdx.x * kHeadSamples;
  const int nb = min(kHeadSamples, B - b0);
  for (int e = threadIdx.x; e < nb * LK; e += 256) {
    const int bl = e / LK, j = e - bl * LK;
    const int l = j / K, k = j - l * K;
    const long b = b0 + bl;
    float v = 0.f;
    for (int ch = 0; ch < pa.chunks[l]; ++ch) v += pa.part[l][(long)ch * M + b * K + k];
    pooled[b * LK + j] = v;
    if (out != nullptr) sh[e] = v * dense_w[j];
  }
  if (out == nullptr) return;
  __syncthreads();
  if (threadIdx.x < nb) {
    float o = 0.f;
    for (int j = 0; j < LK; ++j) o += sh[threadIdx.x * LK + j];
    out[b0 + threadIdx.x] = o + dense_b[0];
  }
}

static __global__ __launch_bounds__(256) void cin_head_bwd_kernel(const float* __restrict__ g, const float* __restrict__ dense_w,
                                                           const float* __restrict__ pooled, float* __restrict__ dP,
                                                           float* __restrict__ part, int B, int LK, int bchunk) {
  __shared__ float red[4][256];
  const int b_lo = blockIdx.x * bchunk, b_hi = min(B, b_lo + bchunk);
  if (LK + 1 <= 64) {
    const int j = threadIdx.x & 63, w = threadIdx.x >> 6;
    float t = 0.f;
    if (j <= LK) {
      const float wj = j < LK ? dense_w[j] : 0.f;
      for (int b = b_lo + w; b < b_hi; b += 4) {
        const float gb = g[b];
        if (j < LK) {
          dP[(long)b * LK + j] = gb * wj;
          t = fmaf(gb, pooled[(long)b * LK + j], t);
        } else {
          t += gb;
        }
      }
    }
    red[w][j] = t;
    __syncthreads();
    if (w == 0 && j <= LK) part[(long)blockIdx.x * (LK + 1) + j] = ((red[0][j] + red[1][j]) + red[2][j]) + red[3][j];
  } else {
    for (int j = threadIdx.x; j <= LK; j += 256) {
      const float wj = j < LK ? dense_w[j] : 0.f;
      float t = 0.f;
      for (int b = b_lo; b < b_hi; ++b) {
        const float gb = g[b];
        if (j < LK) {
          dP[(long)b * LK + j] = gb * wj;
          t = fmaf(gb, pooled[(long)b * LK + j], t);
        } else {
          t += gb;
        }
      }
      part[(long)blockIdx.x * (LK + 1) + j] = t;
    }
  }
}


}
```

ml_function_amd/csrc/cin_layout.h:

```cpp
#pragma once
#include "cin_kernels.h"
#include "cin_tail.h"
#include "cin_launch.h"
#include "cin_qtail.h"
#include "cin_qsplit.h"
#include "cin_qmerge.h"

#include <stdlib.h>

namespace fil {

struct CinShape {
  int B, F, K, L;
  int H[kCinMaxL];
  int Hp(int l) const { return l == 0 ? F : H[l - 1]; }
  int HS(int l) const { return 128 * cdiv(H[l], 128); }
  int xps(int l) const { return l == 0 ? F : HS(l - 1); }
  long M() const { return (long)B * K; }
  int JT() const { return cin_jt_of(F); }
  int HSmax() const {
    int h = 0;
    for (int l = 0; l < L; ++l) h = std::max(h, HS(l));
    return h;
  }
};

static int check_shape(const char* fn, int B, int F, int K, int L, const int* H, CinShape& s) {
  if (B < 0 || F < 1 || K < 1 || L < 1 || H == nullptr) return fail(FIL_ERR_ARG, "%s: bad shape B=%d F=%d K=%d L=%d", fn, B, F, K, L);
  if (L > kCinMaxL) return fail(FIL_ERR_UNSUPPORTED, "%s: L=%d > %d", fn, L, kCinMaxL);
  if (F > kCinMaxFields) return fail(FIL_ERR_UNSUPPORTED, "%s: F=%d > %d fields", fn, F, kCinMaxFields);
  if ((long)B * K > (1L << 28)) return fail(FIL_ERR_UNSUPPORTED, "%s: B*K = %ld rows > 2^28 (row-split byte offsets of the dW kernel are 32-bit)", fn, (long)B * K);
  s.B = B; s.F = F; s.K = K; s.L = L;
  for (int l = 0; l < L; ++l) {
    if (H[l] < 1) return fail(FIL_ERR_ARG, "%s: H[%d]=%d", fn, l, H[l]);
    if (H[l] > kCinMaxH) return fail(FIL_ERR_UNSUPPORTED, "%s: H[%d]=%d > %d feature maps", fn, l, H[l], kCinMaxH);
    s.H[l] = H[l];
  }
  return FIL_OK;
}

static int chunks_of(int H) { return cdiv(H, 128); }
static int env_int(const char* name, int dflt) {
  const char* v = getenv(name);
  return v != nullptr && *v != 0 ? atoi(v) : dflt;
}
struct Knobs {
  int mb, sym, dw_mb, dw_splits, dz_mb, tail_splits, tail_settle, tail_dz_mode, ksplit, dzs_mb, qtail, qmerge, dz2, fwdq, headfold, packfold, dwfold4;
};
static const Knobs& knobs() {
  static const Knobs k = {env_int("FIL_CIN_MB", 0), env_int("FIL_CIN_SYM", 1), env_int("FIL_CIN_DW_MB", 1), env_int("FIL_CIN_DW_SPLITS", 0),
                          env_int("FIL_CIN_DZ_MB", 1), env_int("FIL_CIN_TAIL_SPLITS", 0), env_int("FIL_CIN_TAIL_SETTLE", 0), env_int("FIL_CIN_TAIL_DZ_MODE", 0), env_int("FIL_CIN_KSPLIT", -1), env_int("FIL_CIN_DZS_MB", 0), env_int("FIL_CIN_QTAIL", 1), env_int("FIL_CIN_QMERGE", 1), env_int("FIL_CIN_DZ2", 1), env_int("FIL_CIN_FWDQ", 1), env_int("FIL_CIN_HEADFOLD", 1), env_int("FIL_CIN_PACKFOLD", 1), env_int("FIL_CIN_DWFOLD4", 1)};
  return k;
}
struct CinTune {
  int mb_forced;
  bool sym, no_ksplit;
  CinTune() : CinTune(0) {}
  explicit CinTune(int mode)
      : mb_forced((mode & FIL_CIN_MB2) ? 2 : knobs().mb), sym(knobs().sym != 0 && !(mode & FIL_CIN_NOSYM)), no_ksplit((mode & FIL_CIN_NOKSPLIT) != 0) {}
  int mb_rows(long M) const {
    if (mb_forced == 1 || mb_forced == 2) return mb_forced;
    return cdiv((int)std::min<long>(M, 1L << 30), 64) >= 768 ? 2 : 1;
  }
  int ksplit(long M) const {
    if (knobs().ksplit == 0 || no_ksplit) return 1;
    if (mb_rows(M) != 1) return 1;
    if (knobs().ksplit == 4) return 4;
    return cdiv((int)std::min<long>(M, 1L << 30), 32) <= 512 ? 4 : 1;
  }
};

struct DwPlan {
  int MB, blocks_x, splits, rows_per_split, chunks;
};
static int cu_count() {
  static const int n = [] {
    int dev = 0, v = 0;
    if (hipGetDevice(&dev) != hipSuccess || hipDeviceGetAttribute(&v, hipDeviceAttributeMultiprocessorCount, dev) != hipSuccess || v <= 0) v = 256;
    return v;
  }();
  return n;
}

static DwPlan dw_plan(long M, int C, int H) {
  DwPlan p;
  p.chunks = chunks_of(H);
  p.MB = knobs().dw_mb == 2 ? 2 : 1;
  const int waves_c = cdiv(C, 32 * p.MB);
  p.blocks_x = cdiv(waves_c, 4);
  const long tiles = (long)p.blocks_x * p.chunks;
  const long ncu = cu_count();
  const long unit = 2 * kDwDepth;
  auto rows_of = [&](int splits) { return std::max<long>(unit, ((M + splits - 1) / splits + unit - 1) / unit * unit); };
  int best = knobs().dw_splits;
  if (best <= 0) {
    static const double t_of[4] = {0.0, 1.05e-4, 1.39e-4, 1.96e-4};
    double best_ms = -1.0;
    for (int sp = (int)std::max<long>(1, (M + (1L << 20) - 1) >> 20); sp <= 256; ++sp) {
      const long rps = rows_of(sp);
      const long real = (M + rps - 1) / rps;
      if (real != sp && sp > 1) continue;
      long wgs = tiles * real;
      double per_row = 0.0;
      while (wgs > 0) {
        const long round = std::min(wgs, 3 * ncu);
        per_row += t_of[std::min<long>(3, (round + ncu - 1) / ncu)];
        wgs -= round;
      }
      const double ms = (double)rps * per_row * p.MB + (double)real * C * H * 4.0 / 6e9;
      if (best_ms < 0 || ms < best_ms) best = sp, best_ms = ms;
      if (rps == unit) break;
    }
  }
  best = std::min(std::max(best, 1), 256);
  const long rps = rows_of(best);
  p.rows_per_split = (int)rps;
  p.splits = (int)std::max<long>(1, (M + rps - 1) / rps);
  return p;
}

struct TailGeom {
  bool on = false;
  int p = 0;
  int NCB = 0, JP = 0, JT4 = 0, NQ = 0, JHp = 0;
  int Hpp = 0, Hq = 0, HL = 0, Cp = 0, C1 = 0;
  int periods = 0, tiles = 0;
  size_t uf_floats = 0, uz_floats = 0;
};
static TailGeom tail_geom(const CinShape& s) {
  TailGeom g;
  if (s.L < 3 || !cin_tail_supported(s.F)) return g;
  g.on = true;
  g.p = s.L - 2;
  g.NCB = cin_tail_ncb(s.F);
  g.JP = 16 * g.NCB;
  g.JT4 = cin_tail_jt4(s.F);
  g.NQ = cin_tail_nq(s.F);
  g.JHp = 4 * g.NQ;
  g.Hpp = s.H[g.p - 1];
  g.Hq = s.H[g.p];
  g.HL = s.H[s.L - 1];
  g.Cp = g.Hpp * s.F;
  g.C1 = g.Cp + 1;
  const int JT = s.JT();
  g.periods = cin_dz_periods(g.Hpp, JT);
  g.tiles = cin_slot_tiles(g.Hpp, JT);
  g.uf_floats = (size_t)g.Hpp * g.JT4 * 64 * g.NCB + (size_t)align_up(g.JP + 1, 64);
  g.uz_floats = (size_t)g.tiles * 64 * g.JHp;
  return g;
}
struct TailDwPlan {
  int blocks_x, splits, rows_per_split;
};
static TailDwPlan tail_dw_plan(long M, int C1) {
  TailDwPlan p;
  p.blocks_x = cdiv(C1, 16 * kTailCbw);
  const long unit = 4L * 4 * kTailDwDepth;
  long want = knobs().tail_splits > 0 ? knobs().tail_splits : std::max<long>(1, 2L * cu_count() / p.blocks_x);
  want = std::max<long>(want, (M + (1L << 22) - 1) >> 22);
  const long rows = std::max(unit, ((M + want - 1) / want + unit - 1) / unit * unit);
  p.rows_per_split = (int)rows;
  p.splits = (int)std::max<long>(1, (M + rows - 1) / rows);
  return p;
}

constexpr int kHeadChunk = 16;
constexpr int kColRows = 128;

static size_t wf_floats(const CinShape& s) {
  size_t w = 0;
  for (int l = 0; l < s.L; ++l) {
    w = std::max(w, (size_t)chunks_of(s.H[l]) * s.Hp(l) * 2 * s.JT() * 128);
  }
  w = std::max(w, (size_t)chunks_of(s.H[0]) * s.F * 2 * cin_jt_sym(s.F) * 128);
  w += (size_t)2 * 2 * s.JT() * 128;
  return w;
}
static size_t wz_floats(const CinShape& s) {
  size_t w = (size_t)cin_slot_tiles(s.F, cin_jt_sym(s.F)) * 32 * s.HS(0);
  w = std::max(w, (size_t)s.F * (s.F / 2 + 1) * s.H[0]);
  for (int l = 0; l < s.L; ++l) w = std::max(w, (size_t)cin_slot_tiles(s.Hp(l), s.JT()) * 32 * s.HS(l));
  return w;
}
static int pool_chunks(const CinShape& s, int l) { return std::max(chunks_of(s.H[l]), l > 0 ? chunks_of(s.H[l - 1]) : 1); }
static size_t dw_part_floats(const CinShape& s) {
  size_t pmax = 0;
  for (int l = 0; l < s.L; ++l) pmax = std::max(pmax, (size_t)dw_plan(s.M(), s.Hp(l) * s.F, s.H[l]).splits * s.Hp(l) * s.F * s.H[l]);
  const int csym = s.F * (s.F / 2 + 1);
  pmax = std::max(pmax, (size_t)dw_plan(s.M(), csym, s.H[0]).splits * csym * s.H[0]);
  pmax = std::max(pmax, (size_t)dw_plan(s.M(), csym + s.F, s.H[0]).splits * (csym + s.F) * s.H[0]);
  if (s.L == 3) pmax = std::max(pmax, (size_t)cin_dwq_plan(s.M(), csym + s.F, cu_count()).pairs * (csym + s.F) * 256);
  if (s.L == 3) pmax = std::max(pmax, (size_t)cin_dwqb_plan(s.M(), csym + s.F, cu_count()).splits * (csym + s.F) * 256);
  pmax = std::max(pmax, (size_t)dw_plan(s.M(), s.Hp(s.L - 1), s.F).splits * s.Hp(s.L - 1) * s.F);
  pmax = std::max(pmax, (size_t)dw_plan(s.M(), s.F, s.Hp(s.L - 1)).splits * s.Hp(s.L - 1) * s.F);
  const TailGeom g = tail_geom(s);
  if (g.on) {
    pmax = std::max(pmax, (size_t)tail_dw_plan(s.M(), g.C1).splits * g.C1 * g.JP + (size_t)cdiv(g.Cp, kTailPc) * g.Hq * s.F);
  }
  return pmax;
}

struct LayoutSizer {
  size_t off = 0;
  template <typename T> void sub(T*&, size_t n) { off += n * sizeof(T); }
  void seal() { off = align_up(off, 256); }
  template <typename T> void take(T*& p, size_t n) { sub(p, n), seal(); }
};
struct LayoutCarver {
  char* base;
  size_t off = 0;
  explicit LayoutCarver(const void* p) : base(static_cast<char*>(const_cast<void*>(p))) {}
  template <typename T> void sub(T*& p, size_t n) { p = reinterpret_cast<T*>(base + off), off += n * sizeof(T); }
  void seal() { off = align_up(off, 256); }
  template <typename T> void take(T*& p, size_t n) { sub(p, n), seal(); }
};

enum class SavedForm { plain, tail, qtail };
struct CinSaved {
  float* xT;
  float* maps[kCinMaxL];
  float *Y, *Uz, *Uf, *consts, *bmT;
  float *R, *T, *wsumL, *cvec, *wsumP, *wsnP, *WzT;
  template <class Taker>
  void lay_out(Taker& t, const CinShape& s, const TailGeom& g, SavedForm form) {
    const size_t M = (size_t)s.M();
    t.take(xT, M * s.F);
    const int nmaps = form == SavedForm::qtail ? 1 : (form == SavedForm::tail ? g.p : s.L - 1);
    for (int l = 0; l < nmaps; ++l) t.take(maps[l], M * s.HS(l));
    if (form == SavedForm::qtail) {
      t.sub(R, M * s.HS(0));
      t.sub(T, (size_t)s.F * s.F * s.H[0]);
      t.sub(wsumL, (size_t)s.H[1] * s.F);
      t.sub(cvec, (size_t)128);
      t.sub(wsumP, (size_t)s.H[0] * s.F);
      t.sub(wsnP, (size_t)chunks_of(s.H[0]) * 2 * s.JT() * 128);
      t.sub(WzT, (size_t)cin_slot_tiles(s.F, cin_jt_sym(s.F)) * 32 * s.HS(0));
      t.seal();
    } else if (form == SavedForm::tail) {
      t.take(Y, M * g.JP);
      t.sub(Uz, g.uz_floats);
      t.sub(Uf, g.uf_floats - (size_t)align_up(g.JP + 1, 64));
      t.sub(consts, (size_t)align_up(g.JP + 1, 64));
      t.seal();
      t.take(bmT, (size_t)g.Hq * s.F);
    }
  }
};
static size_t saved_bytes(const CinShape& s) {
  const TailGeom g = tail_geom(s);
  size_t t = 0;
  for (SavedForm form : {SavedForm::plain, SavedForm::tail, SavedForm::qtail}) {
    if ((form != SavedForm::plain && !g.on) || (form == SavedForm::qtail && s.L != 3)) continue;
    LayoutSizer z;
    CinSaved().lay_out(z, s, g, form);
    t = std::max(t, z.off);
  }
  return t;
}

struct CinFwdWs {
  float *pool[kCinMaxL], *wsum, *Wf, *zbias, *x2T, *WfT;
  u32x4* Wb;
  template <class Taker>
  void lay_out(Taker& t, const CinShape& s) {
    const size_t M = (size_t)s.M();
    const int jts = cin_jt_sym(s.F);
    for (int l = 0; l < s.L; ++l) t.take(pool[l], (size_t)pool_chunks(s, l) * M);
    t.take(wsum, (size_t)s.Hp(s.L - 1) * s.F);
    t.take(Wf, wf_floats(s));
    t.take(zbias, (size_t)kCinMaxH);
    t.take(x2T, cin_x2_floats(s.M(), cin_x2_len(s.F)));
    t.take(WfT, (size_t)chunks_of(s.H[0]) * s.F * 2 * jts * 128);
    t.take(Wb, (size_t)cin_qs_steps(s.F, jts) * kQsStageBytes / sizeof(u32x4));
  }
};
static size_t fwd_ws_bytes(const CinShape& s) {
  LayoutSizer z;
  CinFwdWs().lay_out(z, s);
  return z.off;
}

struct CinBwdWs {
  float *dP, *G[2], *part, *small, *wsum, *vlast, *Wz, *dxT, *gx0T, *dT, *dcpart, *hpart;
  u32x4 *Wzb1, *Wzb2;
  template <class Taker>
  void lay_out(Taker& t, const CinShape& s) {
    const size_t M = (size_t)s.M(), LK = (size_t)s.L * s.K, HSmax = (size_t)s.HSmax();
    t.take(dP, (size_t)s.B * LK);
    t.take(G[0], M * HSmax);
    t.take(G[1], M * HSmax);
    t.take(part, dw_part_floats(s));
    t.take(small, std::max(ncol(s) * HSmax, (size_t)nblk(s) * (LK + 1)));
    const size_t cl = (size_t)std::max(s.Hp(s.L - 1), s.L == 3 ? s.H[0] : 0) * s.F;
    t.take(wsum, cl);
    t.take(vlast, cl);
    t.take(Wz, wz_floats(s));
    t.take(dxT, M * s.F);
    t.take(gx0T, M * s.F);
    t.take(dT, (size_t)s.F * s.F * kCinMaxH);
    t.take(dcpart, (ndc(s) + 1) * kQtConst);
    t.take(hpart, ndc(s) * (LK + 1));
    const size_t wzb = (size_t)cin_slot_tiles(s.F, cin_jt_sym(s.F)) * 8 * 3072 / sizeof(u32x4);
    t.take(Wzb1, wzb);
    t.take(Wzb2, wzb);
  }
  static int nblk(const CinShape& s) { return cdiv(std::max(1, s.B), kHeadChunk); }
  static size_t ncol(const CinShape& s) { return ((size_t)s.M() + kColRows - 1) / kColRows; }
  static size_t ndc(const CinShape& s) { return ((size_t)s.M() + 255) / 256; }
  struct Scratch {
    float *xr, *gxR, *dxR;
    int XS;
  };
  Scratch scratch(const CinShape& s, bool qmerge) const {
    const int XS = s.F + (qmerge ? 3 : 1);
    float* gxR = G[1] + (size_t)s.M() * XS;
    return Scratch{G[1], gxR, gxR + (size_t)s.M() * s.F, XS};
  }
};
static size_t bwd_ws_bytes(const CinShape& s) {
  LayoutSizer z;
  CinBwdWs().lay_out(z, s);
  return z.off;
}

}
```

ml_function_amd/csrc/cin_qmerge.h:

```cpp
#pragma once
#include "cin_kernels.h"
#include "cin_launch.h"
#include "cin_qtail.h"

namespace fil {

constexpr int kDwqDepth = 6;
constexpr int kDwqThreads = 512;
struct DwqPlan {
  int tiles, ncol_full, rem, splits, pairs, rows_per_split, wgs_full, wgs;
};
inline int cin_dwq_rem_wgs(int rem, int pairs) { return rem == 0 ? 0 : (rem == 1 ? (pairs + 3) / 4 : (rem == 2 ? (pairs + 1) / 2 : pairs)); }
inline DwqPlan cin_dwq_plan(long M, int C, int cus) {
  DwqPlan p;
  p.tiles = (C + 31) / 32;
  p.ncol_full = p.tiles / 4;
  p.rem = p.tiles % 4;
  const long unit = 2 * kDwqDepth;
  const long slots = cus;
  int best = 1;
  for (int s = 1; s <= 512; ++s) {
    if ((long)p.ncol_full * s + cin_dwq_rem_wgs(p.rem, s) > slots) break;
    best = s;
  }
  long want = std::max<long>(2L * best, (M + (1L << 20) - 1) >> 20);
  long rows = std::max(unit, ((M + want - 1) / want + unit - 1) / unit * unit);
  p.rows_per_split = (int)rows;
  p.splits = (int)std::max<long>(1, (M + rows - 1) / rows);
  p.pairs = (p.splits + 1) / 2;
  p.wgs_full = p.ncol_full * p.pairs;
  p.wgs = p.wgs_full + cin_dwq_rem_wgs(p.rem, p.pairs);
  return p;
}

inline DwqPlan cin_dwq_plan4(long M, int C, int cus) {
  DwqPlan p;
  p.tiles = (C + 31) / 32;
  p.ncol_full = p.tiles / 2;
  p.rem = p.tiles % 2;
  const long unit = 2 * kDwqDepth;
  int best = 1;
  for (int q = 1; q <= 256; ++q) {
    if ((long)p.ncol_full * q + (p.rem ? (q + 1) / 2 : 0) > cus) break;
    best = q;
  }
  long want = std::max<long>(4L * best, (M + (1L << 20) - 1) >> 20);
  long rows = std::max(unit, ((M + want - 1) / want + unit - 1) / unit * unit);
  p.rows_per_split = (int)rows;
  p.splits = (int)std::max<long>(1, (M + rows - 1) / rows);
  p.pairs = (p.splits + 3) / 4;
  p.wgs_full = p.ncol_full * p.pairs;
  p.wgs = p.wgs_full + (p.rem ? (p.pairs + 1) / 2 : 0);
  return p;
}

template <int DEPTH = kDwqDepth, int FOLD = 2>
__global__ __launch_bounds__(kDwqThreads, 2) void cin_dwq_kernel(const float* __restrict__ gT, const float* __restrict__ x1T, int HS, const float* __restrict__ xe,
                                                                int XE, float* __restrict__ part, int M, int F, int symD, int rows_per_split, int splits,
                                                                int ncol_full, int rem, int wgs_full, int wgs) {
  __shared__ float fold[4][128][64];
  const int tid = threadIdx.x, lane = tid & 63, wave = tid >> 6;
  const int r = lane & 31, half = lane >> 5;
  const int Cp = F * symD, C = Cp + F;
  const int item = (blockIdx.x & 7) * (gridDim.x >> 3) + (blockIdx.x >> 3);
  if (item >= wgs) return;
  const int wl = FOLD == 4 ? (wave & 1) : (wave & 3), up = FOLD == 4 ? (wave >> 1) : (wave >> 2);
  int tile, pair;
  bool idle = false;
  if constexpr (FOLD == 4) {
    if (item < wgs_full) {
      tile = (item % ncol_full) * 2 + wl;
      pair = item / ncol_full;
    } else {
      tile = ncol_full * 2;
      pair = 2 * (item - wgs_full) + wl;
    }
  } else if (item < wgs_full) {
    tile = (item % ncol_full) * 4 + wl;
    pair = item / ncol_full;
  } else {
    const int j = item - wgs_full;
    if (rem == 1) {
      tile = ncol_full * 4;
      pair = 4 * j + wl;
    } else if (rem == 2) {
      tile = ncol_full * 4 + (wl & 1);
      pair = 2 * j + (wl >> 1);
    } else {
      tile = ncol_full * 4 + wl;
      pair = j;
      idle = wl == 3;
    }
  }
  tile = __builtin_amdgcn_readfirstlane(tile);
  pair = __builtin_amdgcn_readfirstlane(pair);
  const int split = FOLD * pair + up;
  const int npairs = (splits + FOLD - 1) / FOLD;
  const int c0 = tile * 32;
  const int m_lo = split * rows_per_split;
  const int m_hi = min(M, m_lo + rows_per_split);
  const bool work = !idle && pair < npairs && split < splits && m_lo < m_hi;
  const long mrem = work ? (long)m_hi - m_lo : 0;
  const long mbase = work ? m_lo : 0;
  const __amdgpu_buffer_rsrc_t rg = make_rsrc_uniform(gT + mbase * HS, mrem * HS * 4);
  const __amdgpu_buffer_rsrc_t r1 = make_rsrc_uniform(x1T + mbase * HS, mrem * HS * 4);
  const __amdgpu_buffer_rsrc_t rx = make_rsrc_uniform(xe + mbase * XE, mrem * XE * 4);
  const int c = c0 + r;
  const int cc = c < C ? c : C - 1;
  int hh, ff, sel;
  if (cc < Cp) {
    hh = cc / symD;
    ff = (hh + (cc - hh * symD)) % F;
    sel = 0;
  } else {
    hh = F;
    ff = cc - Cp;
    sel = 1;
  }
  const int ho = (half * XE + hh) * 4, fo = (half * XE + ff) * 4, so = (half * XE + F + 1 + sel) * 4;
  const int go = (half * HS + 4 * r) * 4;
  const int steps = work ? (m_hi - m_lo + 1) >> 1 : 0;
  const int groups = (steps + DEPTH - 1) / DEPTH;

  f32x16 acc[8];
#pragma unroll
  for (int nb = 0; nb < 8; ++nb)
#pragma unroll
    for (int i = 0; i < 16; ++i) acc[nb][i] = 0.f;
  f32x4s qg[DEPTH], q1[DEPTH];
  float qh[DEPTH], qf[DEPTH], qs[DEPTH];
  auto fetch = [&](int s, int d) {
    const int row = 2 * s;
    qg[d] = __builtin_bit_cast(f32x4s, __builtin_amdgcn_raw_buffer_load_b128(rg, go, row * HS * 4, 0));
    q1[d] = __builtin_bit_cast(f32x4s, __builtin_amdgcn_raw_buffer_load_b128(r1, go, row * HS * 4, 0));
    qh[d] = __builtin_bit_cast(float, __builtin_amdgcn_raw_buffer_load_b32(rx, ho, row * XE * 4, 0));
    qf[d] = __builtin_bit_cast(float, __builtin_amdgcn_raw_buffer_load_b32(rx, fo, row * XE * 4, 0));
    qs[d] = __builtin_bit_cast(float, __builtin_amdgcn_raw_buffer_load_b32(rx, so, row * XE * 4, 0));
  };
#pragma unroll
  for (int d = 0; d < DEPTH; ++d) fetch(d, d);
  float ac = qh[0] * qf[0], ac2 = ac * qs[0], an, an2;
#pragma unroll 1
  for (int g = 0; g < groups; ++g) {
#pragma unroll
    for (int d = 0; d < DEPTH; ++d) {
      const f32x4s g4 = qg[d], x4 = q1[d];
      an = qh[(d + 1) % DEPTH] * qf[(d + 1) % DEPTH];
      an2 = an * qs[(d + 1) % DEPTH];
      __builtin_amdgcn_sched_barrier(0);
      acc[0] = mfma32(ac, g4[0], acc[0]);
      acc[1] = mfma32(ac, g4[1], acc[1]);
      acc[2] = mfma32(ac, g4[2], acc[2]);
      acc[3] = mfma32(ac, g4[3], acc[3]);
      acc[4] = mfma32(ac2, x4[0], acc[4]);
      acc[5] = mfma32(ac2, x4[1], acc[5]);
      acc[6] = mfma32(ac2, x4[2], acc[6]);
      acc[7] = mfma32(ac2, x4[3], acc[7]);
      ac = an;
      ac2 = an2;
      __builtin_amdgcn_sched_barrier(0);
      fetch(g * DEPTH + d + DEPTH, d);
      __builtin_amdgcn_sched_barrier(0);
    }
  }
  if constexpr (FOLD == 4) {
    const int slot = (up >> 1) * 2 + wl;
    if (up & 1) {
#pragma unroll
      for (int nb = 0; nb < 8; ++nb)
#pragma unroll
        for (int i = 0; i < 16; ++i) fold[slot][nb * 16 + i][lane] = acc[nb][i];
    }
    __syncthreads();
    if (!(up & 1)) {
#pragma unroll
      for (int nb = 0; nb < 8; ++nb)
#pragma unroll
        for (int i = 0; i < 16; ++i) acc[nb][i] += fold[slot][nb * 16 + i][lane];
    }
    __syncthreads();
    if (up == 2) {
#pragma unroll
      for (int nb = 0; nb < 8; ++nb)
#pragma unroll
        for (int i = 0; i < 16; ++i) fold[wl][nb * 16 + i][lane] = acc[nb][i];
    }
    __syncthreads();
    if (up != 0 || pair >= npairs) return;
#pragma unroll
    for (int nb = 0; nb < 8; ++nb)
#pragma unroll
      for (int i = 0; i < 16; ++i) acc[nb][i] += fold[wl][nb * 16 + i][lane];
  } else {
    if (up == 1) {
#pragma unroll
      for (int nb = 0; nb < 8; ++nb)
#pragma unroll
        for (int i = 0; i < 16; ++i) fold[wl][nb * 16 + i][lane] = acc[nb][i];
    }
    __syncthreads();
    if (up == 1 || idle || pair >= npairs) return;
#pragma unroll
    for (int nb = 0; nb < 8; ++nb)
#pragma unroll
      for (int i = 0; i < 16; ++i) acc[nb][i] += fold[wl][nb * 16 + i][lane];
  }
  float* pout = part + (long)pair * C * 256;
#pragma unroll
  for (int reg = 0; reg < 16; ++reg) {
    const int cr = c0 + mfma32_row(reg, half);
    if (cr < C) {
      float* dst = pout + (long)cr * 256 + 4 * r;
      if (cr < Cp) *reinterpret_cast<float4*>(dst) = make_float4(acc[0][reg], acc[1][reg], acc[2][reg], acc[3][reg]);
      *reinterpret_cast<float4*>(dst + 128) = make_float4(acc[4][reg], acc[5][reg], acc[6][reg], acc[7][reg]);
    }
  }
}

static __global__ __launch_bounds__(256) void cin_reduce_expand_q_kernel(const float* __restrict__ part, int parts, int F, int D, int H1, int H2,
                                                                          float* __restrict__ dW1, float* __restrict__ dT, float* __restrict__ vT,
                                                                          const float* __restrict__ bpart, int nbp, float* __restrict__ dbias1,
                                                                          int nb1, const float* __restrict__ hpart, int nhp, int LK,
                                                                          float* __restrict__ ddw, float* __restrict__ ddb) {
  const int Cp = F * D, C = Cp + F;
  const int nbw = (C + 3) / 4;
  if ((int)blockIdx.x >= nbw + nb1) {
    cin_reduce_body(hpart, ddw, (long)LK + 1, nhp, ddb, (long)LK, (int)blockIdx.x - nbw - nb1);
    return;
  }
  if ((int)blockIdx.x >= nbw) {
    cin_reduce_body(bpart, dbias1, (long)H1, nbp, nullptr, 0, (int)blockIdx.x - nbw);
    return;
  }
  const int lane = threadIdx.x & 63, wave = threadIdx.x >> 6;
  const int c = blockIdx.x * 4 + wave;
  if (c >= C) return;
  const long ps = (long)C * 256;
  const float* p0 = part + (long)c * 256 + 4 * lane;
  f32x4 t[8];
#pragma unroll
  for (int u = 0; u < 8; ++u) t[u] = f32x4{0.f, 0.f, 0.f, 0.f};
  int p = 0;
  for (; p + 7 < parts; p += 8) {
#pragma unroll
    for (int u = 0; u < 8; ++u) t[u] += *reinterpret_cast<const f32x4*>(p0 + (long)(p + u) * ps);
  }
  for (; p < parts; ++p) t[0] += *reinterpret_cast<const f32x4*>(p0 + (long)p * ps);
  const f32x4 v = ((t[0] + t[1]) + (t[2] + t[3])) + ((t[4] + t[5]) + (t[6] + t[7]));
  const int col = 4 * lane, n0 = col & 127;
  const bool second = col >= 128;
  const int H = second ? H2 : H1;
  if (c >= Cp) {
    if (second) {
#pragma unroll
      for (int e = 0; e < 4; ++e)
        if (n0 + e < H2) vT[(long)(c - Cp) * H2 + n0 + e] = v[e];
    }
    return;
  }
  const int h = c / D, d = c - h * D;
  const int f = (h + d) % F;
  float* dst = second ? dT : dW1;
  const bool twin = d != 0 && 2 * d != F;
  float* r0 = dst + ((long)h * F + f) * H + n0;
  float* r1 = dst + ((long)f * F + h) * H + n0;
  if ((H & 3) == 0 && n0 + 3 < H) {
    *reinterpret_cast<f32x4*>(r0) = v;
    if (twin) *reinterpret_cast<f32x4*>(r1) = v;
  } else {
#pragma unroll
    for (int e = 0; e < 4; ++e)
      if (n0 + e < H) {
        r0[e] = v[e];
        if (twin) r1[e] = v[e];
      }
  }
}

constexpr int kXeThreads = 1024;
template <int NP = 3>
static __global__ __launch_bounds__(kXeThreads) void cin_qtail_xe_kernel(const float* __restrict__ xT, const float* __restrict__ dPL,
                                                                  const float* __restrict__ dPp, int ldp, int K, float* __restrict__ xe,
                                                                  float* __restrict__ dcpart, int M, int F, int nscale,
                                                                  const float* __restrict__ g, const float* __restrict__ dense_w,
                                                                  const float* __restrict__ pooled, float* __restrict__ dP, float* __restrict__ hpart,
                                                                  int LK, int lL, int lp, const float* __restrict__ W0, float* __restrict__ Wz,
                                                                  int H0, int JTs, int HS0, int tiles0, int npz = -1,
                                                                  const float* __restrict__ Tq = nullptr, int HT = 0, u32x4* __restrict__ Wzb1 = nullptr,
                                                                  u32x4* __restrict__ Wzb2 = nullptr) {
  extern __shared__ __attribute__((aligned(16))) float smem[];
  if ((int)blockIdx.x >= nscale) {
    if (threadIdx.x >= 256) return;
    if (npz < 0) npz = gridDim.x - nscale;
    const int b = blockIdx.x - nscale;
    if (b < npz) cin_pack_wz_sym_body(W0, Wz, F, H0, JTs, HS0, tiles0, b, npz);
    else {
      const int nq = ((int)gridDim.x - nscale - npz) >> 1, q = b - npz;
      if (q < nq) cin_qs_pack_wz_body<NP>(W0, H0, Wzb1, tiles0, F, JTs, q, nq);
      else if (q < 2 * nq) cin_qs_pack_wz_body<NP>(Tq, HT, Wzb2, tiles0, F, JTs, q - nq, nq);
    }
    return;
  }
  const int nl = g != nullptr ? LK / K : 0;
  const int hl = nl + 1, XE = F + 3;
  const int tid = threadIdx.x;
  const long m0 = (long)blockIdx.x * 256;
  const int nrows = (int)min((long)256, (long)M - m0);
  float* xs = smem;
  float* dls = xs + 256 * F;
  float* dps = dls + 256;
  float* hd = dps + 256;
  {
    const float* src = xT + m0 * F;
    const int n = nrows * F;
    if ((reinterpret_cast<uintptr_t>(xT) & 15) == 0) {
      const int n4 = n >> 2;
      for (int i0 = tid; i0 < n4; i0 += 4 * kXeThreads) {
        float4 v[4];
#pragma unroll
        for (int u = 0; u < 4; ++u) v[u] = i0 + u * kXeThreads < n4 ? reinterpret_cast<const float4*>(src)[i0 + u * kXeThreads] : make_float4(0.f, 0.f, 0.f, 0.f);
#pragma unroll
        for (int u = 0; u < 4; ++u)
          if (i0 + u * kXeThreads < n4) reinterpret_cast<float4*>(xs)[i0 + u * kXeThreads] = v[u];
      }
      for (int i = 4 * n4 + tid; i < n; i += kXeThreads) xs[i] = src[i];
    } else {
      for (int i = tid; i < n; i += kXeThreads) xs[i] = src[i];
    }
    for (int i = n + tid; i < 256 * F; i += kXeThreads) xs[i] = 0.f;
  }
  if (tid < 256) {
    const long m = m0 + tid;
    float dl = 0.f, dp = 0.f;
    if (m < M) {
      const long b = m / K;
      const int k = (int)(m - b * K);
      if (g != nullptr) {
        const float gb = g[b];
        for (int l = 0; l < nl; ++l) {
          const float d = gb * dense_w[l * K + k];
          dP[b * LK + l * K + k] = d;
          hd[tid * hl + l] = gb * pooled[b * LK + l * K + k];
        }
        hd[tid * hl + nl] = k == 0 ? gb : 0.f;
        dl = gb * dense_w[lL * K + k];
        dp = gb * dense_w[lp * K + k];
      } else {
        dl = dPL[b * ldp + k];
        dp = dPp[b * ldp + k];
      }
    } else if (g != nullptr) {
      for (int l = 0; l <= nl; ++l) hd[tid * hl + l] = 0.f;
    }
    dls[tid] = dl;
    dps[tid] = dp;
  }
  __syncthreads();
  __shared__ float cs[4][64];
  if (tid < kXeThreads - 256) {
    constexpr int NT = kXeThreads - 256;
    float* dst = xe + m0 * XE;
    const int n4 = nrows * XE >> 2;
    const float rxe = 1.f / (float)XE;
    for (int i4 = tid; i4 < n4; i4 += NT) {
      int rr = (int)(((float)(4 * i4) + 0.5f) * rxe);
      int c = 4 * i4 - rr * XE;
      float e[4];
#pragma unroll
      for (int u = 0; u < 4; ++u) {
        e[u] = c < F ? xs[rr * F + c] : c == F ? 1.f : c == F + 1 ? dls[rr] : dps[rr];
        if (++c == XE) {
          c = 0;
          ++rr;
        }
      }
      reinterpret_cast<float4*>(dst)[i4] = make_float4(e[0], e[1], e[2], e[3]);
    }
    for (int i = 4 * n4 + tid; i < nrows * XE; i += NT) {
      const int rr = i / XE, c = i - rr * XE;
      dst[i] = c < F ? xs[rr * F + c] : c == F ? 1.f : c == F + 1 ? dls[rr] : dps[rr];
    }
  } else {
    const int t2 = tid - (kXeThreads - 256);
    {
      const int f = t2 & 63, q = t2 >> 6;
      float t0 = 0.f, t1 = 0.f;
      if (f < F) {
        for (int rr = 64 * q; rr < 64 * q + 64; rr += 2) {
          t0 += xs[rr * F + f] * dls[rr];
          t1 += xs[(rr + 1) * F + f] * dls[rr + 1];
        }
      } else if (f < F + 2) {
        const float* dv = f == F ? dls : dps;
        for (int rr = 64 * q; rr < 64 * q + 64; rr += 2) {
          t0 += dv[rr];
          t1 += dv[rr + 1];
        }
      }
      cs[q][f] = t0 + t1;
    }
    if (g != nullptr) {
      const int k0 = (int)(m0 % K);
      for (int j = t2; j <= LK; j += 256) {
        float t = 0.f;
        if (j < LK) {
          const int l = j / K, k = j - l * K;
          for (int rr = (k - k0 + K) % K; rr < 256; rr += K) t += hd[rr * hl + l];
        } else {
          for (int rr = (K - k0) % K; rr < 256; rr += K) t += hd[rr * hl + nl];
        }
        hpart[(long)blockIdx.x * (LK + 1) + j] = t;
      }
    }
  }
  __syncthreads();
  if (tid < F + 2) dcpart[(long)blockIdx.x * kQtConst + tid] = (cs[0][tid] + cs[1][tid]) + (cs[2][tid] + cs[3][tid]);
}

constexpr int kDz2FieldStride = 128 * 2;
inline int cin_dz2_rows(int F, int JT) {
  const int hpp = cin_dz_h_per_period(JT);
  return std::max(cin_dz_sym_rows(F, JT), (F + hpp - 1) / hpp * hpp);
}

__device__ __forceinline__ void cin_dz2_finish(const float* smem, int wave, int lane, int wrow0, int M, int F, int K, const float* __restrict__ dsc, int ldp,
                                               float* __restrict__ dxT, int accumulate, float* __restrict__ dx, const float* __restrict__ cvec) {
  constexpr int FS = kDz2FieldStride;
  const float* img = smem + wave * 32 * 2 + 1;
  const int nrow = min(32, M - wrow0);
  if (dx != nullptr) {
    const int rr = lane & 31;
    const int mm = wrow0 + rr;
    const bool ok = rr < nrow;
    const long mc = ok ? mm : M - 1;
    const long bb = mc / K;
    const int kk = (int)(mc - bb * K);
    const float sc = dsc[bb * ldp + kk];
    float* dxb = dx + (bb * F) * K + kk;
    const float* add = dxT + mc * F;
    for (int f0 = lane >> 5; f0 < F; f0 += 16) {
      float a8[8];
#pragma unroll
      for (int u = 0; u < 8; ++u) a8[u] = accumulate ? add[min(f0 + 2 * u, F - 1)] : 0.f;
#pragma unroll
      for (int u = 0; u < 8; ++u) {
        const int f = f0 + 2 * u;
        if (f < F) {
          const float v = a8[u] + img[f * FS + rr * 2] + sc * cvec[f];
          if (ok) dxb[(long)f * K] = v;
        }
      }
    }
    return;
  }
  float* dst = dxT + (long)wrow0 * F;
  for (int idx = lane; idx < nrow * F; idx += 64) {
    const int rr = idx / F, f = idx - rr * F;
    const float v = img[f * FS + rr * 2];
    dst[idx] = accumulate ? dst[idx] + v : v;
  }
}

template <int JT, int G>
__global__ __launch_bounds__(256, 2) void cin_dz2_kernel(const float* __restrict__ g1T, const float* __restrict__ g2T, int HS,
                                                         const float* __restrict__ dsc, int ldp, int K, const float* __restrict__ Wz1,
                                                         const float* __restrict__ Wz2, const float* __restrict__ xT, float* __restrict__ dxT,
                                                         int accumulate, int M, int F, int H1, int H2, int periods, int FR,
                                                         float* __restrict__ dx, const float* __restrict__ cvec) {
  extern __shared__ __attribute__((aligned(16))) float smem[];
  constexpr int P = JT / gcd_c(16, JT);
  constexpr int HPP = 16 * P / JT;
  constexpr int NQ = 16;
  constexpr int FS = kDz2FieldStride;
  const int tid = threadIdx.x, lane = tid & 63, wave = tid >> 6;
  const int r = lane & 31, half = lane >> 5;
  const int wrow0 = (blockIdx.x * 4 + wave) * 32;
  if (wrow0 >= M) return;
  float* lrow = smem + (wave * 32 + r) * 2;
  const int m = wrow0 + r;
  const bool vq = m < M;
  const long mq = vq ? m : M - 1;
  f32x4s gq[16];
  {
    const f32x4s* grow4 = reinterpret_cast<const f32x4s*>(g1T + mq * HS + half * 64);
#pragma unroll
    for (int s4 = 0; s4 < 16; ++s4) gq[s4] = grow4[s4];
  }
  for (int f0 = half; f0 < FR; f0 += 16) {
    float xt[8];
#pragma unroll
    for (int u = 0; u < 8; ++u) xt[u] = xT[mq * F + min(f0 + 2 * u, F - 1)];
#pragma unroll
    for (int u = 0; u < 8; ++u) {
      const int f = f0 + 2 * u;
      if (f < FR) {
        const int keep = (vq && f < F) ? -1 : 0;
        *reinterpret_cast<float2*>(lrow + f * FS) = make_float2(__builtin_bit_cast(float, __builtin_bit_cast(int, xt[u]) & keep), 0.f);
      }
    }
  }
  float dpl;
  {
    const long bb = mq / K;
    dpl = dsc[bb * ldp + (mq - bb * K)];
  }
  __builtin_amdgcn_wave_barrier();
  const long wbytes = ((long)periods * P + 1) * 32 * 128 * 4;
  const int wo = (r * 128 + half * 64) * 4;
  float greg[64];
  auto to_greg = [&](const f32x4s (&gv4)[16], int Hk, float sc) {
#pragma unroll
    for (int s4 = 0; s4 < 16; ++s4)
#pragma unroll
      for (int e = 0; e < 4; ++e) {
        const int keep = (vq && half * 64 + 4 * s4 + e < Hk) ? -1 : 0;
        const float gv = gv4[s4][e];
        greg[4 * s4 + e] = __builtin_bit_cast(float, __builtin_bit_cast(int, gv) & keep) * sc;
      }
  };
  to_greg(gq, H1, 1.f);

#pragma unroll 1
  for (int pass = 0; pass < 2; ++pass) {
    const float* gT = pass == 0 ? g1T : g2T;
    const int Hk = pass == 0 ? H1 : H2;
    const float sc = pass == 0 ? 1.f : dpl;
    const __amdgpu_buffer_rsrc_t rw = make_rsrc(pass == 0 ? Wz1 : Wz2, wbytes);
    auto ldw = [&](int t, int s4) {
      return __builtin_bit_cast(f32x4s, __builtin_amdgcn_raw_buffer_load_b128(rw, wo + 16 * s4, t * (32 * 128 * 4), 0));
    };
    constexpr int QD = 8;
    f32x4s q[QD];
#pragma unroll
    for (int s4 = 0; s4 < QD; ++s4) q[s4] = ldw(0, s4);
    if (pass == 1) {
      const f32x4s* grow4 = reinterpret_cast<const f32x4s*>(gT + mq * HS + half * 64);
      f32x4s g2[16];
#pragma unroll
      for (int s4 = 0; s4 < 16; ++s4) g2[s4] = grow4[s4];
      to_greg(g2, Hk, sc);
    }
    float gx = 0.f;
    f32x16 dprev;
#pragma unroll
    for (int i = 0; i < 16; ++i) dprev[i] = 0.f;
    float xprev[HPP], xcur[HPP];
#pragma unroll
    for (int hl = 0; hl < HPP; ++hl) xprev[hl] = xcur[hl] = 0.f;
    int hprev = 0;
    float2 lv[G];
    float* la[G];
#pragma unroll
    for (int k = 0; k < G; ++k) {
      lv[k] = make_float2(0.f, 0.f);
      la[k] = lrow;
    }
    float *abase = lrow, *awrap = lrow;
    int symh = 0;
    auto sym_period = [&](int hb) {
      symh = hb + half;
      abase = lrow + symh * FS;
      awrap = abase - F * FS;
    };
    auto slot_fetch = [&](int tp, int rr, int k) {
      const int sp = 16 * tp + rr;
      const int off = sp / JT + 2 * (sp % JT);
      la[k] = (symh >= F - off ? awrap : abase) + off * FS;
      lv[k] = *reinterpret_cast<const float2*>(la[k]);
    };
    auto slot_apply = [&](const f32x16& d, const float (&xpv)[HPP], int hb, int tp, int rr, int k) {
      const int sp = 16 * tp + rr;
      const int hl = sp / JT, j = sp % JT;
      const float dz = d[rr];
      gx = fmaf(dz, lv[k].x, gx);
      la[k][1] = fmaf(dz, xpv[hl], lv[k].y);
      if (j == JT - 1) {
        const float t = lane_halves_sum(gx);
        gx = 0.f;
        if (half == 0) __hip_atomic_fetch_add(lrow + (hb + hl) * FS + 1, t, __ATOMIC_RELAXED, __HIP_MEMORY_SCOPE_WAVEFRONT);
      }
    };
    sym_period(hprev);
#pragma unroll
    for (int k = 0; k < G; ++k) slot_fetch(P - 1, k, k);
#pragma unroll 1
    for (int per = 0; per < periods; ++per) {
      const int hbase = per * HPP;
#pragma unroll
      for (int hl = 0; hl < HPP; ++hl) xcur[hl] = lrow[(hbase + hl) * FS];
#pragma unroll
      for (int tp = 0; tp < P; ++tp) {
        const int t = per * P + tp;
        f32x16 d;
#pragma unroll
        for (int i = 0; i < 16; ++i) d[i] = 0.f;
#pragma unroll
        for (int s4 = 0; s4 < NQ; ++s4) {
          const f32x4s w = q[s4 % QD];
          d = mfma32(w[0], greg[4 * s4 + 0], d);
          d = mfma32(w[1], greg[4 * s4 + 1], d);
          d = mfma32(w[2], greg[4 * s4 + 2], d);
          d = mfma32(w[3], greg[4 * s4 + 3], d);
          q[s4 % QD] = s4 + QD < NQ ? ldw(t, s4 + QD) : ldw(t + 1, s4 + QD - NQ);
          if (s4 % G == G - 1) {
#pragma unroll
            for (int k = 0; k < G; ++k) {
              const int rr = s4 - G + 1 + k;
              if (tp == 0) slot_apply(dprev, xprev, hprev, P - 1, rr, k);
              else slot_apply(dprev, xcur, hbase, tp - 1, rr, k);
            }
            if (s4 < 15) {
#pragma unroll
              for (int k = 0; k < G; ++k) slot_fetch(tp == 0 ? P - 1 : tp - 1, s4 + 1 + k, k);
            } else {
              if (tp == 0) sym_period(hbase);
#pragma unroll
              for (int k = 0; k < G; ++k) slot_fetch(tp, k, k);
            }
            __builtin_amdgcn_sched_barrier(0);
          }
        }
        dprev = d;
      }
#pragma unroll
      for (int hl = 0; hl < HPP; ++hl) xprev[hl] = xcur[hl];
      hprev = hbase;
    }
#pragma unroll
    for (int r0 = 0; r0 < 16; r0 += G) {
#pragma unroll
      for (int k = 0; k < G; ++k) slot_apply(dprev, xprev, hprev, P - 1, r0 + k, k);
      if (r0 + G < 16) {
#pragma unroll
        for (int k = 0; k < G; ++k) slot_fetch(P - 1, r0 + G + k, k);
      }
    }
  }
  __builtin_amdgcn_wave_barrier();
  cin_dz2_finish(smem, wave, lane, wrow0, M, F, K, dsc, ldp, dxT, accumulate, dx, cvec);
}

bool cin_launch_dz2(hipStream_t st, int JT, const float* g1T, const float* g2T, int HS, const float* dsc, int ldp, int K, const float* Wz1,
                    const float* Wz2, const float* xT, float* dxT, int accumulate, int M, int F, int H1, int H2, int periods,
                    float* dx = nullptr, const float* cvec = nullptr);

struct CinHeadFold {
  float* pooled;
  float* out;
  const float* dense_w;
  const float* dense_b;
  int kshift, LK, op, oL;
};

template <int NW>
__device__ __forceinline__ void cin_fwdq_epilogue(f32x16 (&acc)[8], const __amdgpu_buffer_rsrc_t& rx, int vhalf, int wo, int r, int half, int wave, int wrow0,
                                                  const float* __restrict__ bias1, const float* __restrict__ wsn, int JTG, const float* __restrict__ cvec,
                                                  float* __restrict__ x1T, float* __restrict__ RT, int HS, float* __restrict__ pool1,
                                                  float* __restrict__ pool_p, float* __restrict__ pool_L, int M, int F, int H, const CinHeadFold& hf,
                                                  float (&lin_s)[NW][32], float (&pv_s)[NW][3][32]) {
  const int lane = half * 32 + r;
  f32x16 t[4];
#pragma unroll
  for (int nb = 0; nb < 4; ++nb)
#pragma unroll
    for (int i = 0; i < 16; ++i) t[nb][i] = 0.f;
  const __amdgpu_buffer_rsrc_t rs = make_rsrc(wsn, (long)2 * JTG * 128 * 4);
  const __amdgpu_buffer_rsrc_t rc = make_rsrc(cvec, (long)kQtConst * 4);
  float xs4[2][4], cs4[2][4];
  f32x4s ws4[2][4];
  auto ldgroup = [&](int j0, int b) {
#pragma unroll
    for (int u = 0; u < 4; ++u) {
      const int j = __builtin_amdgcn_readfirstlane(j0) + u;
      xs4[b][u] = __builtin_bit_cast(float, __builtin_amdgcn_raw_buffer_load_b32(rx, vhalf, j * 512, 0));
      cs4[b][u] = __builtin_bit_cast(float, __builtin_amdgcn_raw_buffer_load_b32(rc, half * 4, j * 8, 0));
      ws4[b][u] = __builtin_bit_cast(f32x4s, __builtin_amdgcn_raw_buffer_load_b128(rs, wo, j * 1024, 0));
    }
  };
  float lin = 0.f;
  ldgroup(0, 0);
#pragma unroll 1
  for (int j0 = 0; j0 < JTG; j0 += 8) {
    ldgroup(j0 + 4, 1);
#pragma unroll
    for (int u = 0; u < 4; ++u) {
      const bool in = 2 * (j0 + u) + half < F;
      lin = fmaf(in ? xs4[0][u] : 0.f, in ? cs4[0][u] : 0.f, lin);
      const float a = xs4[0][u];
      t[0] = mfma32(a, ws4[0][u][0], t[0]);
      t[1] = mfma32(a, ws4[0][u][1], t[1]);
      t[2] = mfma32(a, ws4[0][u][2], t[2]);
      t[3] = mfma32(a, ws4[0][u][3], t[3]);
    }
    if (j0 + 4 < JTG) {
      ldgroup(j0 + 8, 0);
#pragma unroll
      for (int u = 0; u < 4; ++u) {
        const bool in = 2 * (j0 + 4 + u) + half < F;
        lin = fmaf(in ? xs4[1][u] : 0.f, in ? cs4[1][u] : 0.f, lin);
        const float a = xs4[1][u];
        t[0] = mfma32(a, ws4[1][u][0], t[0]);
        t[1] = mfma32(a, ws4[1][u][1], t[1]);
        t[2] = mfma32(a, ws4[1][u][2], t[2]);
        t[3] = mfma32(a, ws4[1][u][3], t[3]);
      }
    }
  }
  lin = lane_halves_sum(lin);
  if (half == 0) lin_s[wave][r] = lin;
  __builtin_amdgcn_wave_barrier();

  float bv[4];
#pragma unroll
  for (int nb = 0; nb < 4; ++nb) bv[nb] = 4 * r + nb < H ? bias1[4 * r + nb] : 0.f;
  const float cp = cvec[kQtConst + 1], cL = cvec[kQtConst];
#pragma unroll
  for (int reg = 0; reg < 16; ++reg) {
    const int row = mfma32_row(reg, half);
    const int m = wrow0 + row;
    const float a0 = acc[0][reg] + bv[0], a1 = acc[1][reg] + bv[1], a2 = acc[2][reg] + bv[2], a3 = acc[3][reg] + bv[3];
    const float b0 = acc[4][reg], b1 = acc[5][reg], b2 = acc[6][reg], b3 = acc[7][reg];
    if (m < M) {
      *reinterpret_cast<float4*>(x1T + (long)m * HS + 4 * r) = make_float4(a0, a1, a2, a3);
      *reinterpret_cast<float4*>(RT + (long)m * HS + 4 * r) = make_float4(b0, b1, b2, b3);
    }
    float p1 = (a0 + a1) + (a2 + a3);
    float eL = a0 * b0, ep = a0 * t[0][reg];
    eL = fmaf(a1, b1, eL);
    eL = fmaf(a2, b2, eL);
    eL = fmaf(a3, b3, eL);
    ep = fmaf(a1, t[1][reg], ep);
    ep = fmaf(a2, t[2][reg], ep);
    ep = fmaf(a3, t[3][reg], ep);
    p1 = half_wave_sum_hi(p1);
    eL = half_wave_sum_hi(eL);
    ep = half_wave_sum_hi(ep);
    if (r == 31 && m < M) {
      const float vp = ep + cp, vL = (eL + lin_s[wave][row]) + cL;
      if (hf.pooled != nullptr) {
        float* pr = hf.pooled + (long)(m >> hf.kshift) * hf.LK + (m & ((1 << hf.kshift) - 1));
        pr[0] = p1;
        pr[hf.op] = vp;
        pr[hf.oL] = vL;
        pv_s[wave][0][row] = p1;
        pv_s[wave][1][row] = vp;
        pv_s[wave][2][row] = vL;
      } else {
        pool1[m] = p1;
        pool_p[m] = vp;
        pool_L[m] = vL;
      }
    }
  }
  if (hf.out == nullptr) return;
  __builtin_amdgcn_wave_barrier();
  {
    const int k = (wrow0 + r) & ((1 << hf.kshift) - 1);
    const int o0 = half == 0 ? 0 : hf.op;
    pv_s[wave][half][r] *= hf.dense_w[o0 + k];
    if (half == 0) pv_s[wave][2][r] *= hf.dense_w[hf.oL + k];
  }
  __builtin_amdgcn_wave_barrier();
  const int K = 1 << hf.kshift;
  if (lane < (32 >> hf.kshift) && wrow0 + lane * K < M) {
    float o = 0.f;
    for (int l = 0; l < 3; ++l)
      for (int k = 0; k < K; ++k) o += pv_s[wave][l][lane * K + k];
    hf.out[(wrow0 >> hf.kshift) + lane] = o + hf.dense_b[0];
  }
}

template <int JT>
__global__ __launch_bounds__(256, 2) void cin_fwdq_kernel(const float* __restrict__ x2T, int XL, const float* __restrict__ W1f, const float* __restrict__ WTf,
                                                          const float* __restrict__ bias1, const float* __restrict__ wsn, int JTG,
                                                          const float* __restrict__ cvec, float* __restrict__ x1T, float* __restrict__ RT, int HS,
                                                          float* __restrict__ pool1, float* __restrict__ pool_p, float* __restrict__ pool_L, int M, int F,
                                                          int H, CinHeadFold hf) {
  constexpr int DEPTH = JT % 5 == 0 ? 5 : (JT % 4 == 0 ? 4 : (JT % 7 == 0 ? 7 : (JT % 3 == 0 ? 3 : 2)));
  static_assert(JT % DEPTH == 0, "queue depth must divide the steps per h");
  __shared__ float lin_s[4][32];
  __shared__ float pv_s[4][3][32];
  const int tid = threadIdx.x, lane = tid & 63, wave = tid >> 6;
  const int r = lane & 31, half = lane >> 5;
  const int wrow0 = (blockIdx.x * 4 + wave) * 32;
  if (wrow0 >= M) return;
  const int wrow_u = __builtin_amdgcn_readfirstlane(wrow0);
  const __amdgpu_buffer_rsrc_t rx = make_rsrc_uniform(x2T + (long)(wrow_u >> 6) * XL * 64, (long)XL * 256);
  const long wbytes = (long)F * (2 * JT) * 128 * 4;
  const __amdgpu_buffer_rsrc_t rw1 = make_rsrc(W1f, wbytes), rwt = make_rsrc(WTf, wbytes);
  const int wo = (half * 32 + r) * 16;
  const int vrow = ((wrow_u & 63) + r) * 4, vhalf = vrow + half * 256;
  auto ldw = [&](const __amdgpu_buffer_rsrc_t& rw, int s) {
    return __builtin_bit_cast(f32x4s, __builtin_amdgcn_raw_buffer_load_b128(rw, wo, s * 1024, 0));
  };
  auto ldfrag = [&](int h, float (&xf)[JT], float& xp) {
    const int hb = __builtin_amdgcn_readfirstlane(h) * 256;
    xp = __builtin_bit_cast(float, __builtin_amdgcn_raw_buffer_load_b32(rx, vrow, hb, 0));
#pragma unroll
    for (int j = 0; j < JT; ++j) xf[j] = __builtin_bit_cast(float, __builtin_amdgcn_raw_buffer_load_b32(rx, vhalf + 512 * j, hb, 0));
  };
  f32x16 acc[8];
#pragma unroll
  for (int nb = 0; nb < 8; ++nb)
#pragma unroll
    for (int i = 0; i < 16; ++i) acc[nb][i] = 0.f;
  f32x4s q1[DEPTH], qt[DEPTH];
#pragma unroll
  for (int d = 0; d < DEPTH; ++d) {
    q1[d] = ldw(rw1, d);
    qt[d] = ldw(rwt, d);
  }
  float xa[JT], xb[JT], pa, pb;
  ldfrag(0, xa, pa);
#pragma unroll
  for (int d = 0; d < DEPTH; ++d) {
    settle(q1[d]);
    settle(qt[d]);
  }
  settle(pa);
  float ac = pa * xa[0], an;
  auto run_h = [&](int h, float (&xc)[JT], float& pc, float (&xn_)[JT], float& pn) {
    ldfrag(min(h + 1, F - 1), xn_, pn);
    const int sb = h * JT;
#pragma unroll
    for (int j = 0; j < JT; ++j) {
      const f32x4s w1 = q1[j % DEPTH], wt = qt[j % DEPTH];
      an = j + 1 < JT ? pc * xc[j + 1 < JT ? j + 1 : 0] : pn * xn_[0];
      __builtin_amdgcn_sched_barrier(0);
      acc[0] = mfma32(ac, w1[0], acc[0]);
      acc[1] = mfma32(ac, w1[1], acc[1]);
      acc[2] = mfma32(ac, w1[2], acc[2]);
      acc[3] = mfma32(ac, w1[3], acc[3]);
      acc[4] = mfma32(ac, wt[0], acc[4]);
      acc[5] = mfma32(ac, wt[1], acc[5]);
      acc[6] = mfma32(ac, wt[2], acc[6]);
      acc[7] = mfma32(ac, wt[3], acc[7]);
      ac = an;
      __builtin_amdgcn_sched_barrier(0);
      q1[j % DEPTH] = ldw(rw1, sb + j + DEPTH);
      qt[j % DEPTH] = ldw(rwt, sb + j + DEPTH);
      __builtin_amdgcn_sched_barrier(0);
    }
  };
  int h = 0;
#pragma unroll 1
  for (; h + 1 < F; h += 2) {
    run_h(h, xa, pa, xb, pb);
    run_h(h + 1, xb, pb, xa, pa);
  }
  if (h < F) run_h(h, xa, pa, xb, pb);

  cin_fwdq_epilogue<4>(acc, rx, vhalf, wo, r, half, wave, wrow0, bias1, wsn, JTG, cvec, x1T, RT, HS, pool1, pool_p, pool_L, M, F, H, hf, lin_s, pv_s);
}

bool cin_launch_fwdq(hipStream_t st, int JT, const float* x2T, int XL, const float* W1f, const float* WTf, const float* bias1, const float* wsn, int JTG,
                     const float* cvec, float* x1T, float* RT, int HS, float* pool1, float* pool_p, float* pool_L, int M, int F, int H, CinHeadFold hf);

}
```

ml_function_amd/csrc/cin_qmerge.hip:

```cpp
#include "cin_qmerge.h"

namespace fil {

template <int JT, int G>
static void dz2g(hipStream_t st, const float* g1T, const float* g2T, int HS, const float* dsc, int ldp, int K, const float* Wz1, const float* Wz2,
                 const float* xT, float* dxT, int accumulate, int M, int F, int H1, int H2, int periods, float* dx, const float* cvec) {
  const int FR = cin_dz2_rows(F, JT);
  const size_t sh = (size_t)FR * kDz2FieldStride * sizeof(float);
  if (sh > 48 * 1024)
    (void)hipFuncSetAttribute(reinterpret_cast<const void*>(cin_dz2_kernel<JT, G>), hipFuncAttributeMaxDynamicSharedMemorySize, (int)sh);
  hipLaunchKernelGGL((cin_dz2_kernel<JT, G>), dim3(cdiv(M, 128)), dim3(kCinThreads), sh, st, g1T, g2T, HS, dsc, ldp, K, Wz1, Wz2, xT, dxT, accumulate, M, F, H1,
                     H2, periods, FR, dx, cvec);
}
template <int JT>
static void dz2(hipStream_t st, const float* g1T, const float* g2T, int HS, const float* dsc, int ldp, int K, const float* Wz1, const float* Wz2,
                const float* xT, float* dxT, int accumulate, int M, int F, int H1, int H2, int periods, float* dx, const float* cvec) {
  if (JT >= 4 && F >= cin_dz_h_per_period(JT) + 2 * JT) dz2g<JT, (JT >= 4 ? 4 : 1)>(st, g1T, g2T, HS, dsc, ldp, K, Wz1, Wz2, xT, dxT, accumulate, M, F, H1, H2, periods, dx, cvec);
  else dz2g<JT, 1>(st, g1T, g2T, HS, dsc, ldp, K, Wz1, Wz2, xT, dxT, accumulate, M, F, H1, H2, periods, dx, cvec);
}

bool cin_launch_dz2(hipStream_t st, int JT, const float* g1T, const float* g2T, int HS, const float* dsc, int ldp, int K, const float* Wz1,
                    const float* Wz2, const float* xT, float* dxT, int accumulate, int M, int F, int H1, int H2, int periods, float* dx, const float* cvec) {
#define FIL_Z2(JTV) \
  case JTV: dz2<JTV>(st, g1T, g2T, HS, dsc, ldp, K, Wz1, Wz2, xT, dxT, accumulate, M, F, H1, H2, periods, dx, cvec); break;
  switch (JT) { FIL_Z2(2) FIL_Z2(4) FIL_Z2(6) FIL_Z2(8) FIL_Z2(10) FIL_Z2(12) FIL_Z2(14) FIL_Z2(16) FIL_Z2(18) default: return false; }
#undef FIL_Z2
  return true;
}

bool cin_launch_fwdq(hipStream_t st, int JT, const float* x2T, int XL, const float* W1f, const float* WTf, const float* bias1, const float* wsn, int JTG,
                     const float* cvec, float* x1T, float* RT, int HS, float* pool1, float* pool_p, float* pool_L, int M, int F, int H, CinHeadFold hf) {
#define FIL_FQ(JTV)                                                                                                                             \
  case JTV:                                                                                                                                     \
    hipLaunchKernelGGL((cin_fwdq_kernel<JTV>), dim3(cdiv(M, 128)), dim3(kCinThreads), 0, st, x2T, XL, W1f, WTf, bias1, wsn, JTG, cvec, x1T, RT, HS, \
                       pool1, pool_p, pool_L, M, F, H, hf);                                                                                       \
    break;
  switch (JT) { FIL_FQ(2) FIL_FQ(4) FIL_FQ(6) FIL_FQ(8) FIL_FQ(10) FIL_FQ(12) FIL_FQ(14) FIL_FQ(16) FIL_FQ(18) default: return false; }
#undef FIL_FQ
  return true;
}

}
```

Measured before the change: 5.747 million.

## Precompute first-layer gradient factor in forward to skip backward G pass

When head folding, dz2 and the merged forward path are active, the forward kernel writes a per-row gradient factor built from dense weights and layer outputs into the R buffer instead of raw R. The backward pass then uses this with a per-row output-gradient scalar, so last_bwd2 skips its transposed phase and the separate G computation. The dW kernel gains one extra column for the bias-gradient term, and the reduce kernel drops its dedicated bias blocks. This removes a gradient materialisation pass and some memory traffic, at the cost of extra forward epilogue work and more template variants.

New measurement: 5.851 million (median of 6 runs). 1.02x the previous value.

```diff
diff --git a/ml_function_amd/csrc/cin.hip b/ml_function_amd/csrc/cin.hip
--- a/ml_function_amd/csrc/cin.hip
+++ b/ml_function_amd/csrc/cin.hip
@@ -61,6 +61,11 @@
   const CinTune tune(mode);
   return CinPath{(mode & FIL_CIN_X_TRANSPOSED) != 0, (mode & FIL_CIN_GENERAL) != 0, tail_used(s, mode), qtail_used(s, mode, tune), qmerge_used(s, mode, tune),
                  qsplit_used(s, mode, tune), (mode & kCinPrecBf16) != 0 ? 1 : 3, tune, tail_geom(s)};
+}
+static bool cin_ghat_used(const CinShape& s, const CinPath& p, int output_dim) {
+  const bool headfold = output_dim == 1 && s.K <= 32 && (s.K & (s.K - 1)) == 0 && knobs().headfold != 0;
+  const bool dz2 = knobs().dz2 != 0 && s.HS(0) / 2 == 64;
+  return p.qmerge && p.fwdq(s) && !p.qsplit && headfold && dz2 && knobs().ghat != 0;
 }
 static int cin_precision_bits(const char* who, int mode, int precision, int* bits) {
   if (precision != FIL_CIN_PREC_DEFAULT && precision != FIL_CIN_PREC_BF16)
@@ -282,7 +287,7 @@
                              H[0], hf))
         return fail(FIL_ERR_UNSUPPORTED, "fil_cin_fwd: no split-bf16 forward kernel for JT=%d (F=%d)", JTs, F);
     } else if (!cin_launch_fwdq(st, JTs, ws.x2T, XL, ws.Wf, ws.WfT, c.bias[0], sv.wsnP, JT, sv.cvec, x1T, sv.R, HS0, ws.pool[0], ws.pool[p], ws.pool[lL], (int)M, F,
-                                H[0], hf))
+                                H[0], hf, cin_ghat_used(s, c.p, c.output_dim)))
       return fail(FIL_ERR_UNSUPPORTED, "fil_cin_fwd: no merged forward kernel for JT=%d (F=%d)", JTs, F);
     c.pa.chunks[0] = c.pa.chunks[p] = c.pa.chunks[lL] = 1;
   }
@@ -558,11 +563,13 @@
   const int symD = F / 2 + 1, Cl = F * symD;
   const int JTs = cin_jt_sym(F);
   const int periods = cin_dz_periods(F, JTs), tiles0 = cin_slot_tiles(F, JTs);
-  const CinBwdWs::Scratch v = ws.scratch(s, true);
-  float* G = ws.G[c.cur];
+  const bool ghat = cin_ghat_used(s, c.p, c.output_dim);
+  const CinBwdWs::Scratch v = ws.scratch(s, true, ghat);
+  const float* G = ghat ? sv.R : ws.G[c.cur];
+  const float* gsc = ghat ? c.g : nullptr;
   {
     ProfScope ps("cin_tail_a", st, (double)M * (2 * F + 3) * sizeof(float));
-    const size_t sh = (size_t)256 * (F + 3 + (c.output_dim == 1 ? L : 0)) * sizeof(float);
+    const size_t sh = (size_t)256 * (F + 3 + (c.output_dim == 1 ? L : 0) + (ghat ? 1 : 0)) * sizeof(float);
     allow_lds(cin_qtail_xe_kernel<3>, sh);
     allow_lds(cin_qtail_xe_kernel<1>, sh);
     const int np = (int)std::min<long>(((long)tiles0 * 32 * HS0 + 255) / 256, 1024);
@@ -570,16 +577,19 @@
     if (c.p.qnp == 1)
       hipLaunchKernelGGL(cin_qtail_xe_kernel<1>, dim3(c.ndc + np + nq2), dim3(kXeThreads), sh, st, xT, dPL, dPp, LK, K, v.xr, ws.dcpart, (int)M, F,
                          c.ndc, c.output_dim == 1 ? c.g : nullptr, c.dense_w, c.pooled, ws.dP, ws.hpart, LK, lL, p, c.W[0], ws.Wz, H[0], JTs, HS0, tiles0, np, sv.T,
-                         Hpp, ws.Wzb1, ws.Wzb2);
+                         Hpp, ws.Wzb1, ws.Wzb2, ghat ? 1 : 0);
     else
       hipLaunchKernelGGL(cin_qtail_xe_kernel<3>, dim3(c.ndc + np + nq2), dim3(kXeThreads), sh, st, xT, dPL, dPp, LK, K, v.xr, ws.dcpart, (int)M, F,
                          c.ndc, c.output_dim == 1 ? c.g : nullptr, c.dense_w, c.pooled, ws.dP, ws.hpart, LK, lL, p, c.W[0], ws.Wz, H[0], JTs, HS0, tiles0, np, sv.T,
-                         Hpp, ws.Wzb1, ws.Wzb2);
+                         Hpp, ws.Wzb1, ws.Wzb2, ghat ? 1 : 0);
   }
   FIL_CIN_BWD_LAUNCHED();
   {
     ProfScope ps("cin_last_bwd", st, 6.0 * (double)M * Hpp * F);
-    cin_launch_last_bwd2(st, JT, xT, xpT, xps, sv.wsumP, sv.wsnP, dPp, LK, dPprev, G, HS0, ws.dxT, (int)M, F, K, Hpp, sv.R, HS0, dPL, ws.small);
+    if (ghat)
+      cin_launch_last_bwd2(st, JT, xT, xpT, xps, sv.wsumP, sv.wsnP, dPp, LK, nullptr, nullptr, HS0, ws.dxT, (int)M, F, K, Hpp);
+    else
+      cin_launch_last_bwd2(st, JT, xT, xpT, xps, sv.wsumP, sv.wsnP, dPp, LK, dPprev, ws.G[c.cur], HS0, ws.dxT, (int)M, F, K, Hpp, sv.R, HS0, dPL, ws.small);
   }
   FIL_CIN_BWD_LAUNCHED();
   int dw_parts = 0;
@@ -591,23 +601,31 @@
       dw_parts = bp.splits;
     } else {
       const bool f4 = knobs().dwfold4 != 0;
-      const DwqPlan dp = f4 ? cin_dwq_plan4(M, Cl + F, cu_count()) : cin_dwq_plan(M, Cl + F, cu_count());
-      if (f4)
-        hipLaunchKernelGGL((cin_dwq_kernel<kDwqDepth, 4>), dim3((dp.wgs + 7) / 8 * 8), dim3(kDwqThreads), 0, st, G, xpT, HS0, v.xr, v.XS, ws.part, (int)M, F,
-                           symD, dp.rows_per_split, dp.splits, dp.ncol_full, dp.rem, dp.wgs_full, dp.wgs);
-      else
-        hipLaunchKernelGGL((cin_dwq_kernel<kDwqDepth, 2>), dim3((dp.wgs + 7) / 8 * 8), dim3(kDwqThreads), 0, st, G, xpT, HS0, v.xr, v.XS, ws.part, (int)M, F,
-                           symD, dp.rows_per_split, dp.splits, dp.ncol_full, dp.rem, dp.wgs_full, dp.wgs);
+      const int Cw = Cl + F + (ghat ? 1 : 0);
+      const DwqPlan dp = f4 ? cin_dwq_plan4(M, Cw, cu_count()) : cin_dwq_plan(M, Cw, cu_count());
+#define FIL_DWQ(FOLDV, GHV) \
+  hipLaunchKernelGGL((cin_dwq_kernel<kDwqDepth, FOLDV, GHV>), dim3((dp.wgs + 7) / 8 * 8), dim3(kDwqThreads), 0, st, G, xpT, HS0, v.xr, v.XS, ws.part, (int)M, F, \
+                     symD, dp.rows_per_split, dp.splits, dp.ncol_full, dp.rem, dp.wgs_full, dp.wgs)
+      if (ghat) {
+        if (f4) FIL_DWQ(4, true); else FIL_DWQ(2, true);
+      } else {
+        if (f4) FIL_DWQ(4, false); else FIL_DWQ(2, false);
+      }
+#undef FIL_DWQ
       dw_parts = dp.pairs;
     }
   }
   FIL_CIN_BWD_LAUNCHED();
   {
     ProfScope ps("cin_reduce_dw", st);
-    const int nb1 = cdiv(H[0], 64);
+    const int nb1 = ghat ? 0 : cdiv(H[0], 64);
     const int nh = c.output_dim == 1 ? cdiv(LK + 1, 64) : 0;
-    hipLaunchKernelGGL(cin_reduce_expand_q_kernel, dim3((Cl + F + 3) / 4 + nb1 + nh), dim3(256), 0, st, ws.part, dw_parts, F, symD, H[0], Hpp, c.dW[0], ws.dT,
-                       ws.vlast, ws.small, c.ncol, c.dbias[0], nb1, ws.hpart, c.ndc, LK, c.ddense_w, c.ddense_b);
+    if (ghat)
+      hipLaunchKernelGGL(cin_reduce_expand_q_kernel<true>, dim3((Cl + F + 1 + 3) / 4 + nh), dim3(256), 0, st, ws.part, dw_parts, F, symD, H[0], Hpp, c.dW[0], ws.dT,
+                         ws.vlast, ws.small, c.ncol, c.dbias[0], nb1, ws.hpart, c.ndc, LK, c.ddense_w, c.ddense_b);
+    else
+      hipLaunchKernelGGL(cin_reduce_expand_q_kernel<false>, dim3((Cl + F + 3) / 4 + nb1 + nh), dim3(256), 0, st, ws.part, dw_parts, F, symD, H[0], Hpp, c.dW[0], ws.dT,
+                         ws.vlast, ws.small, c.ncol, c.dbias[0], nb1, ws.hpart, c.ndc, LK, c.ddense_w, c.ddense_b);
   }
   FIL_CIN_BWD_LAUNCHED();
   ready_next(c);
@@ -624,7 +642,7 @@
       split_done = cin_launch_dz2_b(st, c.p.qnp, JTs, G, xpT, HS0, dPL, LK, K, ws.Wzb1, ws.Wzb2, xT, ws.dxT, 1, (int)M, F, H[0], Hpp, periods, c.dx, sv.cvec);
     }
     if (!split_done &&
-        !cin_launch_dz2(st, JTs, G, xpT, HS0, dPL, LK, K, ws.Wz, sv.WzT, xT, ws.dxT, 1, (int)M, F, H[0], Hpp, periods, c.dx, sv.cvec))
+        !cin_launch_dz2(st, JTs, G, xpT, HS0, dPL, LK, K, ws.Wz, sv.WzT, xT, ws.dxT, 1, (int)M, F, H[0], Hpp, periods, c.dx, sv.cvec, gsc))
       return fail(FIL_ERR_UNSUPPORTED, "fil_cin_bwd: no two-pass data-gradient kernel for JT=%d (F=%d)", JTs, F);
     c.qm_joined = true;
   } else {
diff --git a/ml_function_amd/csrc/cin_kernels.h b/ml_function_amd/csrc/cin_kernels.h
--- a/ml_function_amd/csrc/cin_kernels.h
+++ b/ml_function_amd/csrc/cin_kernels.h
@@ -1271,6 +1271,7 @@
                                                             float* __restrict__ GprevT, int HSp, float* __restrict__ dxT, int M, int F,
                                                             int K, int Hp, const float* __restrict__ Radd = nullptr, int HSr = 0,
                                                             const float* __restrict__ dPadd = nullptr, float* __restrict__ colpart = nullptr) {
+  const bool do_t = GprevT != nullptr;
   __shared__ float colred[4][128];
   extern __shared__ __attribute__((aligned(16))) float smem[];
   for (int i = threadIdx.x; i < Hp * F; i += 256) smem[i] = wsum[i];
@@ -1282,7 +1283,7 @@
   const long mq = min(wrow0 + r, M - 1);
   float* stg = smem + ((Hp * F + 3) & ~3) + wave * kLast2Stage;
   const int nrow = min(32, M - wrow0);
-  if (nrow > 0) {
+  if (nrow > 0 && do_t) {
     const float4* src = reinterpret_cast<const float4*>(xT + (long)wrow0 * F);
     const int n4 = nrow * F / 4, tail = nrow * F - 4 * n4;
     for (int i = lane; i < n4; i += 64) *reinterpret_cast<float4*>(stg + 4 * i) = src[i];
@@ -1295,7 +1296,7 @@
 #pragma unroll
     for (int j = 0; j < JT; ++j) {
       const int f = 2 * j + half;
-      xr[j] = (f < F && nrow > 0) ? xrow[min(f, F - 1)] : 0.f;
+      xr[j] = (f < F && nrow > 0 && do_t) ? xrow[min(f, F - 1)] : 0.f;
     }
   }
   __shared__ float dps[4][3][32];
@@ -1454,9 +1455,9 @@
     }
   }
   };
-  if ((blockIdx.x >> 3) & 1) {
+  if (!do_t || ((blockIdx.x >> 3) & 1)) {
     phase_u();
-    phase_t();
+    if (do_t) phase_t();
   } else {
     phase_t();
     phase_u();
diff --git a/ml_function_amd/csrc/cin_layout.h b/ml_function_amd/csrc/cin_layout.h
--- a/ml_function_amd/csrc/cin_layout.h
+++ b/ml_function_amd/csrc/cin_layout.h
@@ -45,11 +45,11 @@
   return v != nullptr && *v != 0 ? atoi(v) : dflt;
 }
 struct Knobs {
-  int mb, sym, dw_mb, dw_splits, dz_mb, tail_splits, tail_settle, tail_dz_mode, ksplit, dzs_mb, qtail, qmerge, dz2, fwdq, headfold, packfold, dwfold4;
+  int mb, sym, dw_mb, dw_splits, dz_mb, tail_splits, tail_settle, tail_dz_mode, ksplit, dzs_mb, qtail, qmerge, dz2, fwdq, headfold, packfold, dwfold4, ghat;
 };
 static const Knobs& knobs() {
   static const Knobs k = {env_int("FIL_CIN_MB", 0), env_int("FIL_CIN_SYM", 1), env_int("FIL_CIN_DW_MB", 1), env_int("FIL_CIN_DW_SPLITS", 0),
-                          env_int("FIL_CIN_DZ_MB", 1), env_int("FIL_CIN_TAIL_SPLITS", 0), env_int("FIL_CIN_TAIL_SETTLE", 0), env_int("FIL_CIN_TAIL_DZ_MODE", 0), env_int("FIL_CIN_KSPLIT", -1), env_int("FIL_CIN_DZS_MB", 0), env_int("FIL_CIN_QTAIL", 1), env_int("FIL_CIN_QMERGE", 1), env_int("FIL_CIN_DZ2", 1), env_int("FIL_CIN_FWDQ", 1), env_int("FIL_CIN_HEADFOLD", 1), env_int("FIL_CIN_PACKFOLD", 1), env_int("FIL_CIN_DWFOLD4", 1)};
+                          env_int("FIL_CIN_DZ_MB", 1), env_int("FIL_CIN_TAIL_SPLITS", 0), env_int("FIL_CIN_TAIL_SETTLE", 0), env_int("FIL_CIN_TAIL_DZ_MODE", 0), env_int("FIL_CIN_KSPLIT", -1), env_int("FIL_CIN_DZS_MB", 0), env_int("FIL_CIN_QTAIL", 1), env_int("FIL_CIN_QMERGE", 1), env_int("FIL_CIN_DZ2", 1), env_int("FIL_CIN_FWDQ", 1), env_int("FIL_CIN_HEADFOLD", 1), env_int("FIL_CIN_PACKFOLD", 1), env_int("FIL_CIN_DWFOLD4", 1), env_int("FIL_CIN_GHAT", 1)};
   return k;
 }
 struct CinTune {
@@ -189,7 +189,7 @@
   const int csym = s.F * (s.F / 2 + 1);
   pmax = std::max(pmax, (size_t)dw_plan(s.M(), csym, s.H[0]).splits * csym * s.H[0]);
   pmax = std::max(pmax, (size_t)dw_plan(s.M(), csym + s.F, s.H[0]).splits * (csym + s.F) * s.H[0]);
-  if (s.L == 3) pmax = std::max(pmax, (size_t)cin_dwq_plan(s.M(), csym + s.F, cu_count()).pairs * (csym + s.F) * 256);
+  if (s.L == 3) pmax = std::max(pmax, (size_t)cin_dwq_plan(s.M(), csym + s.F + 1, cu_count()).pairs * (csym + s.F + 1) * 256);
   if (s.L == 3) pmax = std::max(pmax, (size_t)cin_dwqb_plan(s.M(), csym + s.F, cu_count()).splits * (csym + s.F) * 256);
   pmax = std::max(pmax, (size_t)dw_plan(s.M(), s.Hp(s.L - 1), s.F).splits * s.Hp(s.L - 1) * s.F);
   pmax = std::max(pmax, (size_t)dw_plan(s.M(), s.F, s.Hp(s.L - 1)).splits * s.Hp(s.L - 1) * s.F);
@@ -311,8 +311,8 @@
     float *xr, *gxR, *dxR;
     int XS;
   };
-  Scratch scratch(const CinShape& s, bool qmerge) const {
-    const int XS = s.F + (qmerge ? 3 : 1);
+  Scratch scratch(const CinShape& s, bool qmerge, bool ghat = false) const {
+    const int XS = s.F + (qmerge ? (ghat ? 4 : 3) : 1);
     float* gxR = G[1] + (size_t)s.M() * XS;
     return Scratch{G[1], gxR, gxR + (size_t)s.M() * s.F, XS};
   }
diff --git a/ml_function_amd/csrc/cin_qmerge.h b/ml_function_amd/csrc/cin_qmerge.h
--- a/ml_function_amd/csrc/cin_qmerge.h
+++ b/ml_function_amd/csrc/cin_qmerge.h
@@ -54,14 +54,14 @@
   return p;
 }
 
-template <int DEPTH = kDwqDepth, int FOLD = 2>
+template <int DEPTH = kDwqDepth, int FOLD = 2, bool GHAT = false>
 __global__ __launch_bounds__(kDwqThreads, 2) void cin_dwq_kernel(const float* __restrict__ gT, const float* __restrict__ x1T, int HS, const float* __restrict__ xe,
                                                                 int XE, float* __restrict__ part, int M, int F, int symD, int rows_per_split, int splits,
                                                                 int ncol_full, int rem, int wgs_full, int wgs) {
   __shared__ float fold[4][128][64];
   const int tid = threadIdx.x, lane = tid & 63, wave = tid >> 6;
   const int r = lane & 31, half = lane >> 5;
-  const int Cp = F * symD, C = Cp + F;
+  const int Cp = F * symD, C = Cp + F + (GHAT ? 1 : 0);
   const int item = (blockIdx.x & 7) * (gridDim.x >> 3) + (blockIdx.x >> 3);
   if (item >= wgs) return;
   const int wl = FOLD == 4 ? (wave & 1) : (wave & 3), up = FOLD == 4 ? (wave >> 1) : (wave >> 2);
@@ -112,13 +112,17 @@
     hh = cc / symD;
     ff = (hh + (cc - hh * symD)) % F;
     sel = 0;
-  } else {
+  } else if (!GHAT || cc < Cp + F) {
     hh = F;
     ff = cc - Cp;
     sel = 1;
+  } else {
+    hh = ff = F;
+    sel = 1;
   }
   const int ho = (half * XE + hh) * 4, fo = (half * XE + ff) * 4, so = (half * XE + F + 1 + sel) * 4;
   const int go = (half * HS + 4 * r) * 4;
+  const int gso = (half * XE + F + 3) * 4;
   const int steps = work ? (m_hi - m_lo + 1) >> 1 : 0;
   const int groups = (steps + DEPTH - 1) / DEPTH;
 
@@ -128,7 +132,7 @@
 #pragma unroll
     for (int i = 0; i < 16; ++i) acc[nb][i] = 0.f;
   f32x4s qg[DEPTH], q1[DEPTH];
-  float qh[DEPTH], qf[DEPTH], qs[DEPTH];
+  float qh[DEPTH], qf[DEPTH], qs[DEPTH], qgs[DEPTH];
   auto fetch = [&](int s, int d) {
     const int row = 2 * s;
     qg[d] = __builtin_bit_cast(f32x4s, __builtin_amdgcn_raw_buffer_load_b128(rg, go, row * HS * 4, 0));
@@ -136,10 +140,13 @@
     qh[d] = __builtin_bit_cast(float, __builtin_amdgcn_raw_buffer_load_b32(rx, ho, row * XE * 4, 0));
     qf[d] = __builtin_bit_cast(float, __builtin_amdgcn_raw_buffer_load_b32(rx, fo, row * XE * 4, 0));
     qs[d] = __builtin_bit_cast(float, __builtin_amdgcn_raw_buffer_load_b32(rx, so, row * XE * 4, 0));
+    if constexpr (GHAT) qgs[d] = __builtin_bit_cast(float, __builtin_amdgcn_raw_buffer_load_b32(rx, gso, row * XE * 4, 0));
   };
 #pragma unroll
   for (int d = 0; d < DEPTH; ++d) fetch(d, d);
   float ac = qh[0] * qf[0], ac2 = ac * qs[0], an, an2;
+  float ag = ac, ang;
+  if constexpr (GHAT) ag = ac * qgs[0];
 #pragma unroll 1
   for (int g = 0; g < groups; ++g) {
 #pragma unroll
@@ -147,17 +154,20 @@
       const f32x4s g4 = qg[d], x4 = q1[d];
       an = qh[(d + 1) % DEPTH] * qf[(d + 1) % DEPTH];
       an2 = an * qs[(d + 1) % DEPTH];
+      if constexpr (GHAT) ang = an * qgs[(d + 1) % DEPTH];
+      else ang = an;
       __builtin_amdgcn_sched_barrier(0);
-      acc[0] = mfma32(ac, g4[0], acc[0]);
-      acc[1] = mfma32(ac, g4[1], acc[1]);
-      acc[2] = mfma32(ac, g4[2], acc[2]);
-      acc[3] = mfma32(ac, g4[3], acc[3]);
+      acc[0] = mfma32(ag, g4[0], acc[0]);
+      acc[1] = mfma32(ag, g4[1], acc[1]);
+      acc[2] = mfma32(ag, g4[2], acc[2]);
+      acc[3] = mfma32(ag, g4[3], acc[3]);
       acc[4] = mfma32(ac2, x4[0], acc[4]);
       acc[5] = mfma32(ac2, x4[1], acc[5]);
       acc[6] = mfma32(ac2, x4[2], acc[6]);
       acc[7] = mfma32(ac2, x4[3], acc[7]);
       ac = an;
       ac2 = an2;
+      ag = ang;
       __builtin_amdgcn_sched_barrier(0);
       fetch(g * DEPTH + d + DEPTH, d);
       __builtin_amdgcn_sched_barrier(0);
@@ -211,18 +221,19 @@
     const int cr = c0 + mfma32_row(reg, half);
     if (cr < C) {
       float* dst = pout + (long)cr * 256 + 4 * r;
-      if (cr < Cp) *reinterpret_cast<float4*>(dst) = make_float4(acc[0][reg], acc[1][reg], acc[2][reg], acc[3][reg]);
+      if (cr < Cp || (GHAT && cr == C - 1)) *reinterpret_cast<float4*>(dst) = make_float4(acc[0][reg], acc[1][reg], acc[2][reg], acc[3][reg]);
       *reinterpret_cast<float4*>(dst + 128) = make_float4(acc[4][reg], acc[5][reg], acc[6][reg], acc[7][reg]);
     }
   }
 }
 
+template <bool GHAT = false>
 static __global__ __launch_bounds__(256) void cin_reduce_expand_q_kernel(const float* __restrict__ part, int parts, int F, int D, int H1, int H2,
                                                                           float* __restrict__ dW1, float* __restrict__ dT, float* __restrict__ vT,
                                                                           const float* __restrict__ bpart, int nbp, float* __restrict__ dbias1,
                                                                           int nb1, const float* __restrict__ hpart, int nhp, int LK,
                                                                           float* __restrict__ ddw, float* __restrict__ ddb) {
-  const int Cp = F * D, C = Cp + F;
+  const int Cp = F * D, C = Cp + F + (GHAT ? 1 : 0);
   const int nbw = (C + 3) / 4;
   if ((int)blockIdx.x >= nbw + nb1) {
     cin_reduce_body(hpart, ddw, (long)LK + 1, nhp, ddb, (long)LK, (int)blockIdx.x - nbw - nb1);
@@ -250,6 +261,14 @@
   const int col = 4 * lane, n0 = col & 127;
   const bool second = col >= 128;
   const int H = second ? H2 : H1;
+  if (GHAT && c >= Cp + F) {
+    if (!second) {
+#pragma unroll
+      for (int e = 0; e < 4; ++e)
+        if (n0 + e < H1) dbias1[n0 + e] = v[e];
+    }
+    return;
+  }
   if (c >= Cp) {
     if (second) {
 #pragma unroll
@@ -287,7 +306,7 @@
                                                                   int LK, int lL, int lp, const float* __restrict__ W0, float* __restrict__ Wz,
                                                                   int H0, int JTs, int HS0, int tiles0, int npz = -1,
                                                                   const float* __restrict__ Tq = nullptr, int HT = 0, u32x4* __restrict__ Wzb1 = nullptr,
-                                                                  u32x4* __restrict__ Wzb2 = nullptr) {
+                                                                  u32x4* __restrict__ Wzb2 = nullptr, int gcol = 0) {
   extern __shared__ __attribute__((aligned(16))) float smem[];
   if ((int)blockIdx.x >= nscale) {
     if (threadIdx.x >= 256) return;
@@ -302,7 +321,7 @@
     return;
   }
   const int nl = g != nullptr ? LK / K : 0;
-  const int hl = nl + 1, XE = F + 3;
+  const int hl = nl + 1, XE = F + 3 + gcol;
   const int tid = threadIdx.x;
   const long m0 = (long)blockIdx.x * 256;
   const int nrows = (int)min((long)256, (long)M - m0);
@@ -310,6 +329,7 @@
   float* dls = xs + 256 * F;
   float* dps = dls + 256;
   float* hd = dps + 256;
+  float* gs = hd + 256 * hl;
   {
     const float* src = xT + m0 * F;
     const int n = nrows * F;
@@ -331,12 +351,13 @@
   }
   if (tid < 256) {
     const long m = m0 + tid;
-    float dl = 0.f, dp = 0.f;
+    float dl = 0.f, dp = 0.f, gr = 0.f;
     if (m < M) {
       const long b = m / K;
       const int k = (int)(m - b * K);
       if (g != nullptr) {
         const float gb = g[b];
+        gr = gb;
         for (int l = 0; l < nl; ++l) {
           const float d = gb * dense_w[l * K + k];
           dP[b * LK + l * K + k] = d;
@@ -354,6 +375,7 @@
     }
     dls[tid] = dl;
     dps[tid] = dp;
+    if (gcol) gs[tid] = gr;
   }
   __syncthreads();
   __shared__ float cs[4][64];
@@ -368,7 +390,7 @@
       float e[4];
 #pragma unroll
       for (int u = 0; u < 4; ++u) {
-        e[u] = c < F ? xs[rr * F + c] : c == F ? 1.f : c == F + 1 ? dls[rr] : dps[rr];
+        e[u] = c < F ? xs[rr * F + c] : c == F ? 1.f : c == F + 1 ? dls[rr] : c == F + 2 ? dps[rr] : gs[rr];
         if (++c == XE) {
           c = 0;
           ++rr;
@@ -378,7 +400,7 @@
     }
     for (int i = 4 * n4 + tid; i < nrows * XE; i += NT) {
       const int rr = i / XE, c = i - rr * XE;
-      dst[i] = c < F ? xs[rr * F + c] : c == F ? 1.f : c == F + 1 ? dls[rr] : dps[rr];
+      dst[i] = c < F ? xs[rr * F + c] : c == F ? 1.f : c == F + 1 ? dls[rr] : c == F + 2 ? dps[rr] : gs[rr];
     }
   } else {
     const int t2 = tid - (kXeThreads - 256);
@@ -466,7 +488,8 @@
                                                          const float* __restrict__ dsc, int ldp, int K, const float* __restrict__ Wz1,
                                                          const float* __restrict__ Wz2, const float* __restrict__ xT, float* __restrict__ dxT,
                                                          int accumulate, int M, int F, int H1, int H2, int periods, int FR,
-                                                         float* __restrict__ dx, const float* __restrict__ cvec) {
+                                                         float* __restrict__ dx, const float* __restrict__ cvec,
+                                                         const float* __restrict__ gsc = nullptr) {
   extern __shared__ __attribute__((aligned(16))) float smem[];
   constexpr int P = JT / gcd_c(16, JT);
   constexpr int HPP = 16 * P / JT;
@@ -499,10 +522,11 @@
       }
     }
   }
-  float dpl;
+  float dpl, g0;
   {
     const long bb = mq / K;
     dpl = dsc[bb * ldp + (mq - bb * K)];
+    g0 = gsc != nullptr ? gsc[bb] : 1.f;
   }
   __builtin_amdgcn_wave_barrier();
   const long wbytes = ((long)periods * P + 1) * 32 * 128 * 4;
@@ -518,7 +542,7 @@
         greg[4 * s4 + e] = __builtin_bit_cast(float, __builtin_bit_cast(int, gv) & keep) * sc;
       }
   };
-  to_greg(gq, H1, 1.f);
+  to_greg(gq, H1, g0);
 
 #pragma unroll 1
   for (int pass = 0; pass < 2; ++pass) {
@@ -642,7 +666,7 @@
 
 bool cin_launch_dz2(hipStream_t st, int JT, const float* g1T, const float* g2T, int HS, const float* dsc, int ldp, int K, const float* Wz1,
                     const float* Wz2, const float* xT, float* dxT, int accumulate, int M, int F, int H1, int H2, int periods,
-                    float* dx = nullptr, const float* cvec = nullptr);
+                    float* dx = nullptr, const float* cvec = nullptr, const float* gsc = nullptr);
 
 struct CinHeadFold {
   float* pooled;
@@ -652,12 +676,12 @@
   int kshift, LK, op, oL;
 };
 
-template <int NW>
+template <int NW, bool GHAT = false>
 __device__ __forceinline__ void cin_fwdq_epilogue(f32x16 (&acc)[8], const __amdgpu_buffer_rsrc_t& rx, int vhalf, int wo, int r, int half, int wave, int wrow0,
                                                   const float* __restrict__ bias1, const float* __restrict__ wsn, int JTG, const float* __restrict__ cvec,
                                                   float* __restrict__ x1T, float* __restrict__ RT, int HS, float* __restrict__ pool1,
                                                   float* __restrict__ pool_p, float* __restrict__ pool_L, int M, int F, int H, const CinHeadFold& hf,
-                                                  float (&lin_s)[NW][32], float (&pv_s)[NW][3][32]) {
+                                                  float (&lin_s)[NW][32], float (&pv_s)[NW][3][32], float (*gw_s)[3][32] = nullptr) {
   const int lane = half * 32 + r;
   f32x16 t[4];
 #pragma unroll
@@ -708,6 +732,14 @@
   }
   lin = lane_halves_sum(lin);
   if (half == 0) lin_s[wave][r] = lin;
+  if constexpr (GHAT) {
+    const int k = (wrow0 + r) & ((1 << hf.kshift) - 1);
+    if (half == 0) {
+      gw_s[wave][0][r] = hf.dense_w[k];
+      gw_s[wave][1][r] = hf.dense_w[hf.op + k];
+      gw_s[wave][2][r] = hf.dense_w[hf.oL + k];
+    }
+  }
   __builtin_amdgcn_wave_barrier();
 
   float bv[4];
@@ -722,7 +754,7 @@
     const float b0 = acc[4][reg], b1 = acc[5][reg], b2 = acc[6][reg], b3 = acc[7][reg];
     if (m < M) {
       *reinterpret_cast<float4*>(x1T + (long)m * HS + 4 * r) = make_float4(a0, a1, a2, a3);
-      *reinterpret_cast<float4*>(RT + (long)m * HS + 4 * r) = make_float4(b0, b1, b2, b3);
+      if constexpr (!GHAT) *reinterpret_cast<float4*>(RT + (long)m * HS + 4 * r) = make_float4(b0, b1, b2, b3);
     }
     float p1 = (a0 + a1) + (a2 + a3);
     float eL = a0 * b0, ep = a0 * t[0][reg];
@@ -732,6 +764,14 @@
     ep = fmaf(a1, t[1][reg], ep);
     ep = fmaf(a2, t[2][reg], ep);
     ep = fmaf(a3, t[3][reg], ep);
+    if constexpr (GHAT) {
+      const float w1 = gw_s[wave][0][row], wp = gw_s[wave][1][row], wL = gw_s[wave][2][row];
+      const float g0 = 4 * r + 0 < H ? fmaf(wL, b0, fmaf(wp, t[0][reg], w1)) : 0.f;
+      const float g1 = 4 * r + 1 < H ? fmaf(wL, b1, fmaf(wp, t[1][reg], w1)) : 0.f;
+      const float g2 = 4 * r + 2 < H ? fmaf(wL, b2, fmaf(wp, t[2][reg], w1)) : 0.f;
+      const float g3 = 4 * r + 3 < H ? fmaf(wL, b3, fmaf(wp, t[3][reg], w1)) : 0.f;
+      if (m < M) *reinterpret_cast<float4*>(RT + (long)m * HS + 4 * r) = make_float4(g0, g1, g2, g3);
+    }
     p1 = half_wave_sum_hi(p1);
     eL = half_wave_sum_hi(eL);
     ep = half_wave_sum_hi(ep);
@@ -770,7 +810,7 @@
   }
 }
 
-template <int JT>
+template <int JT, bool GHAT = false>
 __global__ __launch_bounds__(256, 2) void cin_fwdq_kernel(const float* __restrict__ x2T, int XL, const float* __restrict__ W1f, const float* __restrict__ WTf,
                                                           const float* __restrict__ bias1, const float* __restrict__ wsn, int JTG,
                                                           const float* __restrict__ cvec, float* __restrict__ x1T, float* __restrict__ RT, int HS,
@@ -780,6 +820,7 @@
   static_assert(JT % DEPTH == 0, "queue depth must divide the steps per h");
   __shared__ float lin_s[4][32];
   __shared__ float pv_s[4][3][32];
+  __shared__ float gw_s[GHAT ? 4 : 1][3][32];
   const int tid = threadIdx.x, lane = tid & 63, wave = tid >> 6;
   const int r = lane & 31, half = lane >> 5;
   const int wrow0 = (blockIdx.x * 4 + wave) * 32;
@@ -850,10 +891,11 @@
   }
   if (h < F) run_h(h, xa, pa, xb, pb);
 
-  cin_fwdq_epilogue<4>(acc, rx, vhalf, wo, r, half, wave, wrow0, bias1, wsn, JTG, cvec, x1T, RT, HS, pool1, pool_p, pool_L, M, F, H, hf, lin_s, pv_s);
+  cin_fwdq_epilogue<4, GHAT>(acc, rx, vhalf, wo, r, half, wave, wrow0, bias1, wsn, JTG, cvec, x1T, RT, HS, pool1, pool_p, pool_L, M, F, H, hf, lin_s, pv_s, gw_s);
 }
 
 bool cin_launch_fwdq(hipStream_t st, int JT, const float* x2T, int XL, const float* W1f, const float* WTf, const float* bias1, const float* wsn, int JTG,
-                     const float* cvec, float* x1T, float* RT, int HS, float* pool1, float* pool_p, float* pool_L, int M, int F, int H, CinHeadFold hf);
-
-}
+                     const float* cvec, float* x1T, float* RT, int HS, float* pool1, float* pool_p, float* pool_L, int M, int F, int H, CinHeadFold hf,
+                     bool ghat = false);
+
+}
diff --git a/ml_function_amd/csrc/cin_qmerge.hip b/ml_function_amd/csrc/cin_qmerge.hip
--- a/ml_function_amd/csrc/cin_qmerge.hip
+++ b/ml_function_amd/csrc/cin_qmerge.hip
@@ -4,36 +4,40 @@
 
 template <int JT, int G>
 static void dz2g(hipStream_t st, const float* g1T, const float* g2T, int HS, const float* dsc, int ldp, int K, const float* Wz1, const float* Wz2,
-                 const float* xT, float* dxT, int accumulate, int M, int F, int H1, int H2, int periods, float* dx, const float* cvec) {
+                 const float* xT, float* dxT, int accumulate, int M, int F, int H1, int H2, int periods, float* dx, const float* cvec, const float* gsc) {
   const int FR = cin_dz2_rows(F, JT);
   const size_t sh = (size_t)FR * kDz2FieldStride * sizeof(float);
   if (sh > 48 * 1024)
     (void)hipFuncSetAttribute(reinterpret_cast<const void*>(cin_dz2_kernel<JT, G>), hipFuncAttributeMaxDynamicSharedMemorySize, (int)sh);
   hipLaunchKernelGGL((cin_dz2_kernel<JT, G>), dim3(cdiv(M, 128)), dim3(kCinThreads), sh, st, g1T, g2T, HS, dsc, ldp, K, Wz1, Wz2, xT, dxT, accumulate, M, F, H1,
-                     H2, periods, FR, dx, cvec);
+                     H2, periods, FR, dx, cvec, gsc);
 }
 template <int JT>
 static void dz2(hipStream_t st, const float* g1T, const float* g2T, int HS, const float* dsc, int ldp, int K, const float* Wz1, const float* Wz2,
-                const float* xT, float* dxT, int accumulate, int M, int F, int H1, int H2, int periods, float* dx, const float* cvec) {
-  if (JT >= 4 && F >= cin_dz_h_per_period(JT) + 2 * JT) dz2g<JT, (JT >= 4 ? 4 : 1)>(st, g1T, g2T, HS, dsc, ldp, K, Wz1, Wz2, xT, dxT, accumulate, M, F, H1, H2, periods, dx, cvec);
-  else dz2g<JT, 1>(st, g1T, g2T, HS, dsc, ldp, K, Wz1, Wz2, xT, dxT, accumulate, M, F, H1, H2, periods, dx, cvec);
+                const float* xT, float* dxT, int accumulate, int M, int F, int H1, int H2, int periods, float* dx, const float* cvec, const float* gsc) {
+  if (JT >= 4 && F >= cin_dz_h_per_period(JT) + 2 * JT) dz2g<JT, (JT >= 4 ? 4 : 1)>(st, g1T, g2T, HS, dsc, ldp, K, Wz1, Wz2, xT, dxT, accumulate, M, F, H1, H2, periods, dx, cvec, gsc);
+  else dz2g<JT, 1>(st, g1T, g2T, HS, dsc, ldp, K, Wz1, Wz2, xT, dxT, accumulate, M, F, H1, H2, periods, dx, cvec, gsc);
 }
 
 bool cin_launch_dz2(hipStream_t st, int JT, const float* g1T, const float* g2T, int HS, const float* dsc, int ldp, int K, const float* Wz1,
-                    const float* Wz2, const float* xT, float* dxT, int accumulate, int M, int F, int H1, int H2, int periods, float* dx, const float* cvec) {
+                    const float* Wz2, const float* xT, float* dxT, int accumulate, int M, int F, int H1, int H2, int periods, float* dx, const float* cvec, const float* gsc) {
 #define FIL_Z2(JTV) \
-  case JTV: dz2<JTV>(st, g1T, g2T, HS, dsc, ldp, K, Wz1, Wz2, xT, dxT, accumulate, M, F, H1, H2, periods, dx, cvec); break;
+  case JTV: dz2<JTV>(st, g1T, g2T, HS, dsc, ldp, K, Wz1, Wz2, xT, dxT, accumulate, M, F, H1, H2, periods, dx, cvec, gsc); break;
   switch (JT) { FIL_Z2(2) FIL_Z2(4) FIL_Z2(6) FIL_Z2(8) FIL_Z2(10) FIL_Z2(12) FIL_Z2(14) FIL_Z2(16) FIL_Z2(18) default: return false; }
 #undef FIL_Z2
   return true;
 }
 
 bool cin_launch_fwdq(hipStream_t st, int JT, const float* x2T, int XL, const float* W1f, const float* WTf, const float* bias1, const float* wsn, int JTG,
-                     const float* cvec, float* x1T, float* RT, int HS, float* pool1, float* pool_p, float* pool_L, int M, int F, int H, CinHeadFold hf) {
-#define FIL_FQ(JTV)                                                                                                                             \
-  case JTV:                                                                                                                                     \
-    hipLaunchKernelGGL((cin_fwdq_kernel<JTV>), dim3(cdiv(M, 128)), dim3(kCinThreads), 0, st, x2T, XL, W1f, WTf, bias1, wsn, JTG, cvec, x1T, RT, HS, \
-                       pool1, pool_p, pool_L, M, F, H, hf);                                                                                       \
+                     const float* cvec, float* x1T, float* RT, int HS, float* pool1, float* pool_p, float* pool_L, int M, int F, int H, CinHeadFold hf, bool ghat) {
+#define FIL_FQ(JTV)                                                                                                                                        \
+  case JTV:                                                                                                                                                \
+    if (ghat)                                                                                                                                              \
+      hipLaunchKernelGGL((cin_fwdq_kernel<JTV, true>), dim3(cdiv(M, 128)), dim3(kCinThreads), 0, st, x2T, XL, W1f, WTf, bias1, wsn, JTG, cvec, x1T, RT, HS, \
+                         pool1, pool_p, pool_L, M, F, H, hf);                                                                                              \
+    else                                                                                                                                                   \
+      hipLaunchKernelGGL((cin_fwdq_kernel<JTV>), dim3(cdiv(M, 128)), dim3(kCinThreads), 0, st, x2T, XL, W1f, WTf, bias1, wsn, JTG, cvec, x1T, RT, HS,      \
+                         pool1, pool_p, pool_L, M, F, H, hf);                                                                                              \
     break;
   switch (JT) { FIL_FQ(2) FIL_FQ(4) FIL_FQ(6) FIL_FQ(8) FIL_FQ(10) FIL_FQ(12) FIL_FQ(14) FIL_FQ(16) FIL_FQ(18) default: return false; }
 #undef FIL_FQ
```
